# abelxiaoxing/ImageClassification

Measured on AMD Instinct MI355X. Metric: images/sec (whole node) ResNet-50 bf16 224^2 training, higher is better.
Workload: dtype bf16; 1 GPU; resnet50 train step, synthetic 3x224x224, batch 256/GPU, AdamW, label smoothing 0.1, 1000 classes (BASELINE configs[1]); global_batch=256, parallelism=dp1

## Files before the change

### imageclassification_amd/csrc/loss_optim.hip

```cpp
#define ICAMD_STREAM_NT 1
#include "common.h"
#include "icamd_internal.h"

namespace {

__global__ __launch_bounds__(256) void softmax_xent_kernel(const bf16_t* __restrict__ logits, int ld, int B, int C,
                                                           const long long* __restrict__ y1, const long long* __restrict__ y2,
                                                           float lam, float smoothing, float gscale,
                                                           float* __restrict__ loss_rows, int* __restrict__ pred,
                                                           bf16_t* __restrict__ dlogits) {
  const int lane = threadIdx.x & 63;
  const int row = blockIdx.x * 4 + (threadIdx.x >> 6);
  if (row >= B) return;
  const bf16_t* x = logits + (long long)row * ld;
  float mx = -INFINITY;
  int amax = lane < C ? lane : 0;
  for (int c = lane; c < C; c += 64) {
    const float v = bf16_to_f32(x[c]);
    if (v > mx) { mx = v; amax = c; }
  }
#pragma unroll
  for (int o = 32; o > 0; o >>= 1) {
    const float om = __shfl_xor(mx, o, 64);
    const int oa = __shfl_xor(amax, o, 64);
    if (om > mx || (om == mx && oa < amax)) { mx = om; amax = oa; }
  }
  float se = 0.f, sx = 0.f;
  for (int c = lane; c < C; c += 64) {
    const float v = bf16_to_f32(x[c]);
    se += __expf(v - mx);
    sx += v;
  }
  se = wave_sum(se);
  sx = wave_sum(sx);
  const float lse = mx + __logf(se);
  const int t1 = (int)y1[row];
  const int t2 = (y2 != nullptr) ? (int)y2[row] : t1;
  const float on = 1.f - smoothing, off = smoothing / (float)C;
  const float lp1 = bf16_to_f32(x[t1]) - lse, lp2 = bf16_to_f32(x[t2]) - lse;
  const float sum_logp = sx - (float)C * lse;
  const float loss = -(off * sum_logp + on * (lam * lp1 + (1.f - lam) * lp2));
  if (lane == 0) {
    loss_rows[row] = loss;
    if (pred != nullptr) pred[row] = amax;
  }
  if (dlogits != nullptr) {
    bf16_t* d = dlogits + (long long)row * ld;
    const float inv = 1.f / se;
    for (int c = lane; c < ld; c += 64) {
      float g = 0.f;
      if (c < C) {
        const float pc = __expf(bf16_to_f32(x[c]) - mx) * inv;
        float t = off;
        if (c == t1) t += on * lam;
        if (c == t2) t += on * (1.f - lam);
        g = (pc - t) * gscale;
      }
      d[c] = f32_to_bf16(g);
    }
  }
}

__global__ __launch_bounds__(256) void step_metrics_kernel(const float* __restrict__ loss_rows,
                                                           const int* __restrict__ pred,
                                                           const long long* __restrict__ target, int B, int C,
                                                           float* __restrict__ loss_out, int* __restrict__ finite_out,
                                                           double* __restrict__ acc_f64, int* __restrict__ counts,
                                                           float* __restrict__ loss_log, int log_slot, int log_stride,
                                                           int respect_skip) {
  __shared__ double red[256];
  __shared__ int cred[256];
  __shared__ int s_finite;
  const bool have_loss = loss_rows != nullptr;
  if (have_loss) {
    double s = 0.0;
    for (int i = threadIdx.x; i < B; i += 256) s += (double)loss_rows[i];
    red[threadIdx.x] = s;
    __syncthreads();
    for (int o = 128; o > 0; o >>= 1) {
      if ((int)threadIdx.x < o) red[threadIdx.x] += red[threadIdx.x + o];
      __syncthreads();
    }
    if (threadIdx.x == 0) {
      const float mean = (float)(red[0] / (double)B);
      const int fin = isfinite(mean) ? 1 : 0;
      *loss_out = mean;
      *finite_out = fin;
      s_finite = fin;
      if (loss_log != nullptr) loss_log[log_slot] = mean;
    }
  } else if (threadIdx.x == 0) {
    s_finite = *finite_out;
  }
  __syncthreads();
  if (respect_skip & 2) return;
  if ((respect_skip & 1) && !s_finite) return;
  const bool add_loss = have_loss || (respect_skip & 4);
  if (pred == nullptr) {
    if (threadIdx.x == 0 && add_loss) { acc_f64[0] += (double)*loss_out; acc_f64[1] += 1.0; }
    return;
  }
  int correct = 0;
  for (int i = threadIdx.x; i < B; i += 256) {
    const int p = pred[i];
    const int t = (int)target[i];
    if (p == t) {
      ++correct;
      if (counts != nullptr && t >= 0 && t < C) atomicAdd(&counts[t], 1);
    } else if (counts != nullptr) {
      if (p >= 0 && p < C) atomicAdd(&counts[C + p], 1);
      if (t >= 0 && t < C) atomicAdd(&counts[2 * C + t], 1);
    }
  }
  cred[threadIdx.x] = correct;
  __syncthreads();
  for (int o = 128; o > 0; o >>= 1) {
    if ((int)threadIdx.x < o) cred[threadIdx.x] += cred[threadIdx.x + o];
    __syncthreads();
  }
  if (threadIdx.x == 0) {
    if (add_loss) { acc_f64[0] += (double)*loss_out; acc_f64[1] += 1.0; }
    acc_f64[2] += (double)((float)cred[0] / (float)B);
    if (loss_log != nullptr && log_stride > 0) loss_log[log_stride + log_slot] = (float)cred[0] / (float)B;
    acc_f64[3] += (double)cred[0];
    acc_f64[4] += (double)B;
  }
}

__global__ __launch_bounds__(256) void sumsq_partial_kernel(const float* __restrict__ g, long long n4, long long n,
                                                            double* __restrict__ partial) {
  __shared__ double red[4];
  const long long stride = (long long)gridDim.x * blockDim.x;
  double s = 0.0;
  for (long long i = (long long)blockIdx.x * blockDim.x + threadIdx.x; i < n4; i += stride) {
    const f32x4 v = ((const f32x4*)g)[i];
    s += (double)(v[0] * v[0] + v[1] * v[1]) + (double)(v[2] * v[2] + v[3] * v[3]);
  }
  if (blockIdx.x == 0 && threadIdx.x == 0)
    for (long long i = n4 * 4; i < n; ++i) s += (double)g[i] * (double)g[i];
  s = wave_sum_d(s);
  if ((threadIdx.x & 63) == 0) red[threadIdx.x >> 6] = s;
  __syncthreads();
  if (threadIdx.x == 0) partial[blockIdx.x] = red[0] + red[1] + red[2] + red[3];
}

__global__ void gradnorm_finalize_kernel(const double* __restrict__ partial, int nblk, float inv_scale, float max_norm,
                                         float* __restrict__ out) {
  if (threadIdx.x != 0 || blockIdx.x != 0) return;
  double s = 0.0;
  for (int i = 0; i < nblk; ++i) s += partial[i];
  const float norm = (float)sqrt(s) * inv_scale;
  out[0] = norm;
  float coef = 1.f;
  if (max_norm > 0.f) { coef = max_norm / (norm + 1e-6f); if (coef > 1.f) coef = 1.f; }
  out[1] = coef;
}

struct AdamArgs {
  float lr, wd, beta1, beta2, eps, gscale, ema_w;
  int step;
  int bias_correct;
};

__device__ __forceinline__ void bias_corrections(const AdamArgs& a, const int* __restrict__ skipped, float& bc1,
                                                 float& bc2_sqrt) {
  bc1 = 1.f; bc2_sqrt = 1.f;
  if (a.bias_correct) {
    int t = a.step - (skipped != nullptr ? *skipped : 0);
    if (t < 1) t = 1;
    bc1 = (float)(1.0 - pow((double)a.beta1, (double)t));
    bc2_sqrt = (float)sqrt(1.0 - pow((double)a.beta2, (double)t));
  }
}
__device__ __forceinline__ bool step_skipped(const int* __restrict__ finite_flag, int* __restrict__ skipped, int flags) {
  if (finite_flag == nullptr || *finite_flag != 0) return false;
  if (skipped != nullptr && !(flags & 2) && blockIdx.x == 0 && threadIdx.x == 0) *skipped += 1;
  return true;
}

__global__ __launch_bounds__(256) void adamw_ema_kernel(float* __restrict__ p, float* __restrict__ g, float* __restrict__ m,
                                                        float* __restrict__ v, float* __restrict__ ema,
                                                        bf16_t* __restrict__ shadow, long long n4, AdamArgs a,
                                                        const float* __restrict__ clip, const int* __restrict__ finite_flag,
                                                        int* __restrict__ skipped, int zero_grad) {
  if (step_skipped(finite_flag, skipped, zero_grad)) return;
  float bc1, bc2_sqrt;
  bias_corrections(a, skipped, bc1, bc2_sqrt);
  const float gs = a.gscale * (clip != nullptr ? clip[1] : 1.f);
  const float decay_mul = 1.f - a.lr * a.wd;
  const float step_size = a.lr / bc1;
  const long long stride = (long long)gridDim.x * blockDim.x;
  for (long long i = (long long)blockIdx.x * blockDim.x + threadIdx.x; i < n4; i += stride) {
    f32x4 pv = ld_stream((const f32x4*)p + i);
    f32x4 gv = ld_stream((const f32x4*)g + i);
    f32x4 mv = ld_stream((const f32x4*)m + i);
    f32x4 vv = ld_stream((const f32x4*)v + i);
#pragma unroll
    for (int e = 0; e < 4; ++e) {
      const float gg = gv[e] * gs;
      float pp = pv[e] * decay_mul;
      const float mm = mv[e] + (gg - mv[e]) * (1.f - a.beta1);
      const float v2 = vv[e] * a.beta2 + (1.f - a.beta2) * gg * gg;
      const float denom = sqrtf(v2) / bc2_sqrt + a.eps;
      pp = pp - step_size * (mm / denom);
      pv[e] = pp; mv[e] = mm; vv[e] = v2;
    }
    ((f32x4*)p)[i] = pv;
    ((f32x4*)m)[i] = mv;
    ((f32x4*)v)[i] = vv;
    if (zero_grad & 1) ((f32x4*)g)[i] = f32x4{0.f, 0.f, 0.f, 0.f};
    if (ema != nullptr) {
      f32x4 ev = ld_stream((const f32x4*)ema + i);
#pragma unroll
      for (int e = 0; e < 4; ++e) ev[e] = ev[e] + a.ema_w * (pv[e] - ev[e]);
      ((f32x4*)ema)[i] = ev;
    }
    if (shadow != nullptr) {
      u32x2 sv;
      sv[0] = pack_bf16x2(pv[0], pv[1]);
      sv[1] = pack_bf16x2(pv[2], pv[3]);
      ((u32x2*)shadow)[i] = sv;
    }
  }
}

__global__ __launch_bounds__(256) void grad_guard_kernel(float* __restrict__ g, long long n4, const int* __restrict__ finite_flag) {
  if (*finite_flag != 0) return;
  const long long stride = (long long)gridDim.x * blockDim.x;
  for (long long i = (long long)blockIdx.x * blockDim.x + threadIdx.x; i < n4; i += stride)
    ((f32x4*)g)[i] = f32x4{0.f, 0.f, 0.f, 0.f};
}

__global__ __launch_bounds__(256) void lerp_kernel(float* __restrict__ dst, const float* __restrict__ src, long long n,
                                                   float w, const int* __restrict__ finite_flag) {
  if (finite_flag != nullptr && *finite_flag == 0) return;
  const long long stride = (long long)gridDim.x * blockDim.x;
  if (w == 1.f) {
    for (long long i = (long long)blockIdx.x * blockDim.x + threadIdx.x; i < n; i += stride) dst[i] = src[i];
    return;
  }
  for (long long i = (long long)blockIdx.x * blockDim.x + threadIdx.x; i < n; i += stride)
    dst[i] = dst[i] + w * (src[i] - dst[i]);
}

__global__ __launch_bounds__(256) void f32_to_bf16_kernel(const float* __restrict__ src, bf16_t* __restrict__ dst,
                                                          long long n) {
  const long long stride = (long long)gridDim.x * blockDim.x;
  for (long long i = (long long)blockIdx.x * blockDim.x + threadIdx.x; i < n; i += stride) dst[i] = f32_to_bf16(src[i]);
}

__global__ __launch_bounds__(256) void filter_transpose_kernel(const bf16_t* __restrict__ src_base,
                                                               bf16_t* __restrict__ dst_base,
                                                               const long long* __restrict__ descs,
                                                               const int* __restrict__ jobs) {
  const int layer = jobs[blockIdx.x * 2 + 0];
  const int start = jobs[blockIdx.x * 2 + 1];
  const long long* d = descs + (long long)layer * 8;
  const bf16_t* src = src_base + d[0];
  bf16_t* dst = dst_base + d[1];
  const int Cout = (int)d[2], T = (int)d[3], Cin = (int)d[4];
  const int total = Cout * T * Cin;
  for (int k = 0; k < 16; ++k) {
    const int o = start + k * 256 + threadIdx.x;
    if (o < total) {
      const int co = o % Cout;
      const int rest = o / Cout;
      const int t = rest % T;
      const int ci = rest / T;
      dst[o] = src[((long long)co * T + t) * Cin + ci];
    }
  }
}

__global__ __launch_bounds__(256) void filter_transpose_tiled_kernel(const bf16_t* __restrict__ src_base,
                                                                     bf16_t* __restrict__ dst_base,
                                                                     const long long* __restrict__ descs,
                                                                     const int* __restrict__ jobs) {
  __shared__ bf16_t tile[64][72];
  const int* job = jobs + blockIdx.x * 4;
  const long long* d = descs + (long long)job[0] * 8;
  const int t = job[1], co0 = job[2], ci0 = job[3];
  const int Cout = (int)d[2], T = (int)d[3], Cin = (int)d[4];
  const bf16_t* src = src_base + d[0];
  bf16_t* dst = dst_base + d[1];
  const int r = threadIdx.x >> 3, c8 = (threadIdx.x & 7) * 8;
#pragma unroll
  for (int pass = 0; pass < 2; ++pass) {
    const int co = r + pass * 32;
    const u32x4 v = *(const u32x4*)(src + ((long long)(co0 + co) * T + t) * Cin + ci0 + c8);
    *(u32x4*)&tile[co][c8] = v;
  }
  __syncthreads();
#pragma unroll
  for (int pass = 0; pass < 2; ++pass) {
    const int ci = r + pass * 32;
    unsigned int w[4];
#pragma unroll
    for (int e = 0; e < 4; ++e)
      w[e] = (unsigned int)tile[c8 + 2 * e][ci] | ((unsigned int)tile[c8 + 2 * e + 1][ci] << 16);
    *(u32x4*)(dst + ((long long)(ci0 + ci) * T + t) * Cout + co0 + c8) = u32x4{w[0], w[1], w[2], w[3]};
  }
}

__global__ __launch_bounds__(256) void colsum_kernel(const bf16_t* __restrict__ x, int rows, int ld, int cols,
                                                     float* __restrict__ out, int accumulate) {
  const int c = blockIdx.x * blockDim.x + threadIdx.x;
  if (c >= cols) return;
  float s = 0.f;
  for (int r = 0; r < rows; ++r) s += bf16_to_f32(x[(long long)r * ld + c]);
  out[c] = accumulate ? out[c] + s : s;
}

inline unsigned int grid_for(long long work_items, int threads) {
  long long blocks = (work_items + threads - 1) / threads;
  if (blocks > 2048) blocks = 2048;
  if (blocks < 1) blocks = 1;
  return (unsigned int)blocks;
}

}

int icamd_softmax_xent_launch(const bf16_t* logits, int ld, int B, int C, const long long* y1, const long long* y2,
                              float lam, float smoothing, float gscale, float* loss_rows, int* pred, bf16_t* dlogits,
                              hipStream_t s) {
  if (B <= 0 || C <= 0 || ld < C) return ICAMD_ERR_BAD_ARG;
  hipLaunchKernelGGL(softmax_xent_kernel, dim3((unsigned)((B + 3) / 4)), dim3(256), 0, s, logits, ld, B, C, y1, y2, lam,
                     smoothing, gscale, loss_rows, pred, dlogits);
  return icamd_launch_status();
}

int icamd_step_metrics_launch(const float* loss_rows, const int* pred, const long long* target, int B, int C,
                              float* loss_out, int* finite_out, double* acc_f64, int* counts, float* loss_log,
                              int log_slot, int log_stride, int respect_skip, hipStream_t s) {
  hipLaunchKernelGGL(step_metrics_kernel, dim3(1), dim3(256), 0, s, loss_rows, pred, target, B, C, loss_out, finite_out,
                     acc_f64, counts, loss_log, log_slot, log_stride, respect_skip);
  return icamd_launch_status();
}

#define ICAMD_SUMSQ_BLOCKS 512
int icamd_grad_norm_launch(const float* g, long long n, float inv_scale, float max_norm, double* partial, float* out,
                           hipStream_t s) {
  const long long n4 = n / 4;
  hipLaunchKernelGGL(sumsq_partial_kernel, dim3(ICAMD_SUMSQ_BLOCKS), dim3(256), 0, s, g, n4, n, partial);
  hipLaunchKernelGGL(gradnorm_finalize_kernel, dim3(1), dim3(64), 0, s, partial, ICAMD_SUMSQ_BLOCKS, inv_scale, max_norm,
                     out);
  return icamd_launch_status();
}

int icamd_adamw_ema_launch(float* p, float* g, float* m, float* v, float* ema, bf16_t* shadow, long long n, float lr,
                           float wd, float beta1, float beta2, float eps, int step, float gscale, float ema_decay,
                           const float* clip, const int* finite_flag, int* skipped, int zero_grad, hipStream_t s) {
  if (n % 4 != 0 || step < 1) return ICAMD_ERR_BAD_ARG;
  AdamArgs a;
  a.lr = lr; a.wd = wd; a.beta1 = beta1; a.beta2 = beta2; a.eps = eps; a.gscale = gscale;
  a.step = step; a.bias_correct = 1;
  a.ema_w = 1.f - ema_decay;
  hipLaunchKernelGGL(adamw_ema_kernel, dim3(grid_for(n / 4, 256)), dim3(256), 0, s, p, g, m, v, ema, shadow, n / 4, a, clip,
                     finite_flag, skipped, zero_grad);
  return icamd_launch_status();
}

int icamd_grad_guard_launch(float* g, long long n, const int* finite_flag, hipStream_t s) {
  if (n % 4 != 0) return ICAMD_ERR_BAD_ARG;
  hipLaunchKernelGGL(grad_guard_kernel, dim3(grid_for(n / 4, 256)), dim3(256), 0, s, g, n / 4, finite_flag);
  return icamd_launch_status();
}

template <int KIND>
__global__ __launch_bounds__(256) void optim_ema_kernel(float* __restrict__ p, float* __restrict__ g, float* __restrict__ m,
                                                        float* __restrict__ v, float* __restrict__ ema,
                                                        bf16_t* __restrict__ shadow, long long n4, AdamArgs a,
                                                        const float* __restrict__ clip, const int* __restrict__ finite_flag,
                                                        int* __restrict__ skipped, int zero_grad) {
  if (step_skipped(finite_flag, skipped, zero_grad)) return;
  float bc1, bc2_sqrt;
  bias_corrections(a, skipped, bc1, bc2_sqrt);
  const float gs = a.gscale * (clip != nullptr ? clip[1] : 1.f);
  const float step_size = a.lr / bc1;
  const long long stride = (long long)gridDim.x * blockDim.x;
  for (long long i = (long long)blockIdx.x * blockDim.x + threadIdx.x; i < n4; i += stride) {
    f32x4 pv = ((f32x4*)p)[i];
    const f32x4 gv = ((const f32x4*)g)[i];
    f32x4 mv = ((f32x4*)m)[i];
    f32x4 vv = {0.f, 0.f, 0.f, 0.f};
    if (KIND == 1) vv = ((f32x4*)v)[i];
#pragma unroll
    for (int e = 0; e < 4; ++e) {
      float gg = gv[e] * gs;
      if (KIND == 1) {
        gg += a.wd * pv[e];
        const float mm = mv[e] + (gg - mv[e]) * (1.f - a.beta1);
        const float v2 = vv[e] * a.beta2 + (1.f - a.beta2) * gg * gg;
        pv[e] -= step_size * (mm / (sqrtf(v2) / bc2_sqrt + a.eps));
        mv[e] = mm; vv[e] = v2;
      } else if (KIND == 2 || KIND == 3) {
        gg += a.wd * pv[e];
        const float buf = a.beta1 * mv[e] + gg;
        pv[e] -= a.lr * (KIND == 3 ? gg + a.beta1 * buf : buf);
        mv[e] = buf;
      } else {
        const float u = mv[e] * a.beta1 + gg * (1.f - a.beta1);
        const float sg = u > 0.f ? 1.f : (u < 0.f ? -1.f : 0.f);
        pv[e] = pv[e] * (1.f - a.lr * a.wd) - a.lr * sg;
        mv[e] = mv[e] + (gg - mv[e]) * (1.f - a.beta2);
      }
    }
    ((f32x4*)p)[i] = pv;
    ((f32x4*)m)[i] = mv;
    if (KIND == 1) ((f32x4*)v)[i] = vv;
    if (zero_grad & 1) ((f32x4*)g)[i] = f32x4{0.f, 0.f, 0.f, 0.f};
    if (ema != nullptr) {
      f32x4 ev = ld_stream((const f32x4*)ema + i);
#pragma unroll
      for (int e = 0; e < 4; ++e) ev[e] = ev[e] + a.ema_w * (pv[e] - ev[e]);
      ((f32x4*)ema)[i] = ev;
    }
    if (shadow != nullptr) {
      u32x2 sv;
      sv[0] = pack_bf16x2(pv[0], pv[1]);
      sv[1] = pack_bf16x2(pv[2], pv[3]);
      ((u32x2*)shadow)[i] = sv;
    }
  }
}

int icamd_optim_ema_launch(int kind, float* p, float* g, float* m, float* v, float* ema, bf16_t* shadow, long long n,
                           float lr, float wd, float beta1, float beta2, float eps, int step, float gscale,
                           float ema_decay, const float* clip, const int* finite_flag, int* skipped, int zero_grad,
                           hipStream_t s) {
  if (kind == 0) return icamd_adamw_ema_launch(p, g, m, v, ema, shadow, n, lr, wd, beta1, beta2, eps, step, gscale, ema_decay,
                                               clip, finite_flag, skipped, zero_grad, s);
  if (n % 4 != 0 || step < 1 || kind < 0 || kind > 4 || (kind == 1 && v == nullptr)) return ICAMD_ERR_BAD_ARG;
  AdamArgs a;
  a.lr = lr; a.wd = wd; a.beta1 = beta1; a.beta2 = beta2; a.eps = eps; a.gscale = gscale;
  a.step = step; a.bias_correct = kind == 1 ? 1 : 0;
  a.ema_w = 1.f - ema_decay;
  const dim3 grid(grid_for(n / 4, 256)), block(256);
  if (kind == 1) hipLaunchKernelGGL(optim_ema_kernel<1>, grid, block, 0, s, p, g, m, v, ema, shadow, n / 4, a, clip, finite_flag, skipped, zero_grad);
  else if (kind == 2) hipLaunchKernelGGL(optim_ema_kernel<2>, grid, block, 0, s, p, g, m, v, ema, shadow, n / 4, a, clip, finite_flag, skipped, zero_grad);
  else if (kind == 3) hipLaunchKernelGGL(optim_ema_kernel<3>, grid, block, 0, s, p, g, m, v, ema, shadow, n / 4, a, clip, finite_flag, skipped, zero_grad);
  else hipLaunchKernelGGL(optim_ema_kernel<4>, grid, block, 0, s, p, g, m, v, ema, shadow, n / 4, a, clip, finite_flag, skipped, zero_grad);
  return icamd_launch_status();
}

int icamd_lerp_launch(float* dst, const float* src, long long n, float w, const int* finite_flag, hipStream_t s) {
  hipLaunchKernelGGL(lerp_kernel, dim3(grid_for(n, 256)), dim3(256), 0, s, dst, src, n, w, finite_flag);
  return icamd_launch_status();
}

int icamd_f32_to_bf16_launch(const float* src, bf16_t* dst, long long n, hipStream_t s) {
  hipLaunchKernelGGL(f32_to_bf16_kernel, dim3(grid_for(n, 256)), dim3(256), 0, s, src, dst, n);
  return icamd_launch_status();
}

int icamd_filter_transpose_launch(const bf16_t* src_base, bf16_t* dst_base, const long long* descs, const int* jobs,
                                  int njobs, hipStream_t s) {
  if (njobs <= 0) return ICAMD_OK;
  hipLaunchKernelGGL(filter_transpose_kernel, dim3((unsigned)njobs), dim3(256), 0, s, src_base, dst_base, descs, jobs);
  return icamd_launch_status();
}

int icamd_filter_transpose_tiled_launch(const bf16_t* src_base, bf16_t* dst_base, const long long* descs, const int* jobs,
                                        int njobs, hipStream_t s) {
  if (njobs <= 0) return ICAMD_OK;
  hipLaunchKernelGGL(filter_transpose_tiled_kernel, dim3((unsigned)njobs), dim3(256), 0, s, src_base, dst_base, descs, jobs);
  return icamd_launch_status();
}

int icamd_colsum_launch(const bf16_t* x, int rows, int ld, int cols, float* out, int accumulate, hipStream_t s) {
  hipLaunchKernelGGL(colsum_kernel, dim3((unsigned)((cols + 255) / 256)), dim3(256), 0, s, x, rows, ld, cols, out,
                     accumulate);
  return icamd_launch_status();
}
```

### imageclassification_amd/csrc/norm_pool.hip

```cpp
#include "common.h"
#include "icamd_internal.h"
#include <stdlib.h>
#include <string.h>

#ifndef ICAMD_BN_NT
#define ICAMD_BN_NT 1
#endif

namespace {

__device__ __forceinline__ u32x4 bn_ld(const void* base, long long i) {
  if constexpr (ICAMD_BN_NT & 1) return __builtin_nontemporal_load((const u32x4*)base + i);
  else return ((const u32x4*)base)[i];
}
__device__ __forceinline__ void bn_st(void* base, long long i, const u32x4 v) {
  if constexpr (ICAMD_BN_NT & 2) __builtin_nontemporal_store(v, (u32x4*)base + i);
  else ((u32x4*)base)[i] = v;
}

__global__ void bn_eval_coeffs_kernel(int C, const float* __restrict__ gamma, const float* __restrict__ beta,
                                      const float* __restrict__ running_mean, const float* __restrict__ running_var,
                                      float eps, float* __restrict__ scale_out, float* __restrict__ shift_out) {
  const int c = blockIdx.x * blockDim.x + threadIdx.x;
  if (c >= C) return;
  const float invstd = 1.0f / sqrtf(running_var[c] + eps);
  const float sc = gamma[c] * invstd;
  scale_out[c] = sc;
  shift_out[c] = beta[c] - running_mean[c] * sc;
}

struct BnFinalizeArgs {
  const float* gamma; const float* beta; float* running_mean; float* running_var;
  float momentum, eps;
  float* mean_out; float* invstd_out; float* scale_out; float* shift_out;
  float* dgamma; float* dbeta; float* c1_out; float* c2_out; int accumulate;
  const float* gy_mean; const float* gy_invstd;
  double count;
};

template <int MODE, int CG>
__global__ __launch_bounds__(1024) void bn_reduce_finalize_kernel(const float* __restrict__ part, double* __restrict__ chunks,
                                                                  unsigned int* __restrict__ counters, int nrows, int C,
                                                                  int rows_per_chunk, BnFinalizeArgs a) {
  constexpr int RL = 1024 / CG;
  __shared__ double red[RL][2][CG];
  __shared__ int s_last;
  const int cc = threadIdx.x & (CG - 1);
  const int c = blockIdx.x * CG + cc;
  const int rl = threadIdx.x / CG;
  const int r0 = blockIdx.y * rows_per_chunk;
  const int r1 = min(nrows, r0 + rows_per_chunk);
  double s1 = 0.0, s2 = 0.0;
  if (c < C) {
    double u1 = 0.0, u2 = 0.0;
    int r = r0 + rl;
    constexpr int UN = 8;
    for (; r + (2 * UN - 1) * RL < r1; r += 2 * UN * RL) {
      float a0[UN], a1[UN], b0[UN], b1[UN];
#pragma unroll
      for (int k = 0; k < UN; ++k) {
        a0[k] = part[((long long)(r + 2 * k * RL) * 2 + 0) * C + c];
        a1[k] = part[((long long)(r + 2 * k * RL) * 2 + 1) * C + c];
        b0[k] = part[((long long)(r + (2 * k + 1) * RL) * 2 + 0) * C + c];
        b1[k] = part[((long long)(r + (2 * k + 1) * RL) * 2 + 1) * C + c];
      }
#pragma unroll
      for (int k = 0; k < UN; ++k) { s1 += (double)a0[k]; s2 += (double)a1[k]; u1 += (double)b0[k]; u2 += (double)b1[k]; }
    }
    for (; r + RL < r1; r += 2 * RL) {
      const float a0 = part[((long long)r * 2 + 0) * C + c], a1 = part[((long long)r * 2 + 1) * C + c];
      const float b0 = part[((long long)(r + RL) * 2 + 0) * C + c], b1 = part[((long long)(r + RL) * 2 + 1) * C + c];
      s1 += (double)a0; s2 += (double)a1; u1 += (double)b0; u2 += (double)b1;
    }
    if (r < r1) { s1 += (double)part[((long long)r * 2 + 0) * C + c]; s2 += (double)part[((long long)r * 2 + 1) * C + c]; }
    s1 += u1; s2 += u2;
  }
  red[rl][0][cc] = s1;
  red[rl][1][cc] = s2;
  __syncthreads();
  double t1 = 0.0, t2 = 0.0;
  if (gridDim.y == 1) {
    if (threadIdx.x >= CG || c >= C) return;
#pragma unroll
    for (int j = 0; j < RL; ++j) { t1 += red[j][0][cc]; t2 += red[j][1][cc]; }
  } else {
  if (threadIdx.x < 2 * CG) {
    const int which = threadIdx.x / CG;
    double s = 0.0;
#pragma unroll
    for (int j = 0; j < RL; ++j) s += red[j][which][cc];
    if (c < C) chunks[((long long)blockIdx.y * 2 + which) * C + c] = s;
  }
  asm volatile("s_waitcnt vmcnt(0)" ::: "memory");
  __syncthreads();
  if (threadIdx.x == 0) {
    __builtin_amdgcn_fence(__ATOMIC_RELEASE, "agent");
    asm volatile("s_waitcnt vmcnt(0)" ::: "memory");
    const unsigned int prev = __hip_atomic_fetch_add(&counters[blockIdx.x], 1u, __ATOMIC_RELAXED, __HIP_MEMORY_SCOPE_AGENT);
    const int last = (prev == gridDim.y - 1) ? 1 : 0;
    if (last) {
      __builtin_amdgcn_fence(__ATOMIC_ACQUIRE, "agent");
      asm volatile("s_waitcnt vmcnt(0)" ::: "memory");
      __hip_atomic_store(&counters[blockIdx.x], 0u, __ATOMIC_RELAXED, __HIP_MEMORY_SCOPE_AGENT);
    }
    s_last = last;
  }
  __syncthreads();
  if (!s_last) return;
  const int nchunks = gridDim.y;
  double p1 = 0.0, p2 = 0.0;
  if (c < C) {
    for (int k = rl; k < nchunks; k += RL) {
      p1 += chunks[((long long)k * 2 + 0) * C + c];
      p2 += chunks[((long long)k * 2 + 1) * C + c];
    }
  }
  red[rl][0][cc] = p1;
  red[rl][1][cc] = p2;
  __syncthreads();
  if (threadIdx.x >= CG || c >= C) return;
#pragma unroll
  for (int j = 0; j < RL; ++j) { t1 += red[j][0][cc]; t2 += red[j][1][cc]; }
  }
  if constexpr (MODE == 0) {
    const double mean = t1 / a.count;
    double var = t2 / a.count - mean * mean;
    if (var < 0.0) var = 0.0;
    const float invstd = (float)(1.0 / sqrt(var + (double)a.eps));
    const float meanf = (float)mean;
    a.mean_out[c] = meanf;
    a.invstd_out[c] = invstd;
    const float sc = a.gamma[c] * invstd;
    a.scale_out[c] = sc;
    a.shift_out[c] = a.beta[c] - meanf * sc;
    if (a.running_mean != nullptr) {
      const double unbiased = a.count > 1.0 ? var * (a.count / (a.count - 1.0)) : var;
      a.running_mean[c] = (1.f - a.momentum) * a.running_mean[c] + a.momentum * meanf;
      a.running_var[c] = (1.f - a.momentum) * a.running_var[c] + a.momentum * (float)unbiased;
    }
  } else {
    if (a.gy_mean != nullptr) t2 = (double)a.gy_invstd[c] * (t2 - (double)a.gy_mean[c] * t1);
    a.c1_out[c] = (float)(t1 / a.count);
    a.c2_out[c] = (float)(t2 / a.count);
    if (a.accumulate) { a.dgamma[c] += (float)t2; a.dbeta[c] += (float)t1; }
    else { a.dgamma[c] = (float)t2; a.dbeta[c] = (float)t1; }
  }
}

__global__ __launch_bounds__(256) void bn_apply_kernel(const bf16_t* __restrict__ y, const float* __restrict__ scale,
                                                       const float* __restrict__ shift, const bf16_t* __restrict__ residual,
                                                       bf16_t* __restrict__ out, unsigned char* __restrict__ maskbits,
                                                       long long nvec, int cpr, int relu,
                                                       const float* __restrict__ res_scale,
                                                       const float* __restrict__ res_shift) {
  const long long stride = (long long)gridDim.x * blockDim.x;
  long long i = (long long)blockIdx.x * blockDim.x + threadIdx.x;
  const int cg = (int)(i % cpr) * 8;
  float sc[8], sh[8], rsc[8], rsh[8];
#pragma unroll
  for (int e = 0; e < 8; ++e) { sc[e] = scale[cg + e]; sh[e] = shift[cg + e]; }
  const bool res_bn = res_scale != nullptr;
#pragma unroll
  for (int e = 0; e < 8; ++e) { rsc[e] = res_bn ? res_scale[cg + e] : 1.f; rsh[e] = res_bn ? res_shift[cg + e] : 0.f; }
  for (; i < nvec; i += stride) {
    const u32x4 v = bn_ld(y, i);
    float f[8];
#pragma unroll
    for (int e = 0; e < 4; ++e) {
      f[2 * e] = fmaf(bf16_lo(v[e]), sc[2 * e], sh[2 * e]);
      f[2 * e + 1] = fmaf(bf16_hi(v[e]), sc[2 * e + 1], sh[2 * e + 1]);
    }
    if (residual != nullptr) {
      const u32x4 r = bn_ld(residual, i);
      if (res_bn) {
#pragma unroll
        for (int e = 0; e < 4; ++e) {
          f[2 * e] += bf16_to_f32(f32_to_bf16(fmaf(bf16_lo(r[e]), rsc[2 * e], rsh[2 * e])));
          f[2 * e + 1] += bf16_to_f32(f32_to_bf16(fmaf(bf16_hi(r[e]), rsc[2 * e + 1], rsh[2 * e + 1])));
        }
      } else {
#pragma unroll
        for (int e = 0; e < 4; ++e) { f[2 * e] += bf16_lo(r[e]); f[2 * e + 1] += bf16_hi(r[e]); }
      }
    }
    if (relu) {
#pragma unroll
      for (int e = 0; e < 8; ++e) f[e] = (f[e] < 0.f) ? 0.f : f[e];
    }
    u32x4 o;
#pragma unroll
    for (int e = 0; e < 4; ++e) o[e] = pack_bf16x2(f[2 * e], f[2 * e + 1]);
    bn_st(out, i, o);
    if (maskbits != nullptr) {
      unsigned int bits = 0;
#pragma unroll
      for (int e = 0; e < 8; ++e) bits |= (f[e] > 0.f ? 1u : 0u) << e;
      maskbits[i] = (unsigned char)bits;
    }
  }
}

struct PoolGather {
  const unsigned char* idx;
  int IH, IW, OH, OW;
  FastDiv dIW, dIH;
};

__device__ __forceinline__ u32x4 pool_gather8(const bf16_t* __restrict__ dout, const PoolGather& pg, unsigned int row,
                                              unsigned int cpr, unsigned int cg) {
  const unsigned int t1 = fdiv(row, pg.dIW);
  const int w = (int)(row - t1 * pg.IW);
  const unsigned int n = fdiv(t1, pg.dIH);
  const int h = (int)(t1 - n * pg.IH);
  float acc[8];
#pragma unroll
  for (int e = 0; e < 8; ++e) acc[e] = 0.f;
  const int oh_lo = h >> 1, oh_hi = (h + 1) >> 1, ow_lo = w >> 1, ow_hi = (w + 1) >> 1;
  for (int oh = oh_lo; oh <= oh_hi; ++oh) {
    if (oh >= pg.OH) continue;
    const int r = h - (oh * 2 - 1);
    for (int ow = ow_lo; ow <= ow_hi; ++ow) {
      if (ow >= pg.OW) continue;
      const unsigned int code4 = (unsigned)(r * 3 + (w - (ow * 2 - 1))) * 0x01010101u;
      const unsigned int o = ((n * pg.OH + oh) * pg.OW + ow) * cpr + cg;
      const u32x2 iv = ((const u32x2*)pg.idx)[o];
      const u32x4 d = ((const u32x4*)dout)[o];
      const unsigned int m0 = iv[0] ^ code4, m1 = iv[1] ^ code4;
#pragma unroll
      for (int e = 0; e < 8; ++e) {
        const unsigned int mb = ((e < 4 ? m0 : m1) >> ((e & 3) * 8)) & 0xffu;
        const float dv = (e & 1) ? bf16_hi(d[e >> 1]) : bf16_lo(d[e >> 1]);
        acc[e] += mb == 0u ? dv : 0.f;
      }
    }
  }
  u32x4 out;
#pragma unroll
  for (int e = 0; e < 4; ++e) out[e] = pack_bf16x2(acc[2 * e], acc[2 * e + 1]);
  return out;
}

__global__ __launch_bounds__(256) void bn_bwd_reduce_kernel(const bf16_t* __restrict__ dout, const bf16_t* __restrict__ act,
                                                            const bf16_t* __restrict__ y, const float* __restrict__ mean,
                                                            const float* __restrict__ invstd, const float* __restrict__ scale,
                                                            const float* __restrict__ shift, float* __restrict__ part,
                                                            const unsigned char* __restrict__ maskbits, long long rows, int C,
                                                            int rows_per_block, int relu, const PoolGather pg) {
  __shared__ float red[256 * 16];
  const int cpr = C >> 3;
  const int tid = threadIdx.x;
  const long long r0 = (long long)blockIdx.x * rows_per_block;
  const long long r1 = (rows < r0 + rows_per_block) ? rows : r0 + rows_per_block;
  for (int cg0 = 0; cg0 < cpr; cg0 += 256) {
    const int tcols = (cpr - cg0 < 256) ? (cpr - cg0) : 256;
    const int rlanes = 256 / tcols;
    const int cgi = tid % tcols, rl = tid / tcols;
    float sg[8], sgx[8];
#pragma unroll
    for (int e = 0; e < 8; ++e) { sg[e] = 0.f; sgx[e] = 0.f; }
    if (rl < rlanes) {
      const int c = (cg0 + cgi) * 8;
      float mu[8], is[8], sc[8], sh[8];
#pragma unroll
      for (int e = 0; e < 8; ++e) { mu[e] = mean[c + e]; is[e] = invstd[c + e]; sc[e] = scale[c + e]; sh[e] = shift[c + e]; }
      for (long long r = r0 + rl; r < r1; r += rlanes) {
        const long long off = r * cpr + cg0 + cgi;
        const u32x4 d = pg.idx != nullptr ? pool_gather8(dout, pg, (unsigned)r, (unsigned)cpr, (unsigned)(cg0 + cgi))
                                          : bn_ld(dout, off);
        const u32x4 yv = bn_ld(y, off);
        float g[8], yy[8];
#pragma unroll
        for (int e = 0; e < 4; ++e) {
          g[2 * e] = bf16_lo(d[e]); g[2 * e + 1] = bf16_hi(d[e]);
          yy[2 * e] = bf16_lo(yv[e]); yy[2 * e + 1] = bf16_hi(yv[e]);
        }
        if (relu) {
          if (maskbits != nullptr) {
            const unsigned int bits = maskbits[off];
#pragma unroll
            for (int e = 0; e < 8; ++e)
              if (!((bits >> e) & 1u)) g[e] = 0.f;
          } else if (act != nullptr) {
            const u32x4 a = bn_ld(act, off);
#pragma unroll
            for (int e = 0; e < 4; ++e) {
              if (!(bf16_lo(a[e]) > 0.f)) g[2 * e] = 0.f;
              if (!(bf16_hi(a[e]) > 0.f)) g[2 * e + 1] = 0.f;
            }
          } else {
#pragma unroll
            for (int e = 0; e < 8; ++e)
              if (!(fmaf(yy[e], sc[e], sh[e]) > 0.f)) g[e] = 0.f;
          }
        }
#pragma unroll
        for (int e = 0; e < 8; ++e) {
          sg[e] += g[e];
          sgx[e] += g[e] * ((yy[e] - mu[e]) * is[e]);
        }
      }
    }
#pragma unroll
    for (int e = 0; e < 8; ++e) { red[tid * 16 + e] = sg[e]; red[tid * 16 + 8 + e] = sgx[e]; }
    __syncthreads();
    for (int o = tid; o < tcols * 16; o += 256) {
      const int cgo = o >> 4, e = o & 15;
      float s = 0.f;
      for (int l = 0; l < rlanes; ++l) s += red[(l * tcols + cgo) * 16 + e];
      const int which = e >> 3;
      part[((long long)blockIdx.x * 2 + which) * C + (cg0 + cgo) * 8 + (e & 7)] = s;
    }
    __syncthreads();
  }
}

__global__ __launch_bounds__(256) void bn_bwd_apply_kernel(const bf16_t* __restrict__ dout, const bf16_t* __restrict__ act,
                                                           const bf16_t* __restrict__ y, const float* __restrict__ mean,
                                                           const float* __restrict__ invstd, const float* __restrict__ scale,
                                                           const float* __restrict__ shift, const float* __restrict__ c1,
                                                           const float* __restrict__ c2, bf16_t* __restrict__ dy,
                                                           bf16_t* __restrict__ gout, const unsigned char* __restrict__ maskbits,
                                                           long long nvec, int cpr, int relu, int reverse,
                                                           const PoolGather pg, const FastDiv dcpr) {
  const long long stride = (long long)gridDim.x * blockDim.x;
  long long k0 = (long long)blockIdx.x * blockDim.x + threadIdx.x;
  const int cg = (int)((reverse ? nvec - 1 - k0 : k0) % cpr) * 8;
  float mu[8], is[8], sc[8], sh[8], k1[8], k2[8];
#pragma unroll
  for (int e = 0; e < 8; ++e) {
    mu[e] = mean[cg + e]; is[e] = invstd[cg + e]; sc[e] = scale[cg + e]; sh[e] = shift[cg + e];
    k1[e] = c1[cg + e]; k2[e] = c2[cg + e];
  }
  for (; k0 < nvec; k0 += stride) {
    const long long i = reverse ? nvec - 1 - k0 : k0;
    u32x4 d;
    if (pg.idx != nullptr) {
      const unsigned int row = fdiv((unsigned)i, dcpr);
      d = pool_gather8(dout, pg, row, (unsigned)cpr, (unsigned)i - row * (unsigned)cpr);
    } else {
      d = bn_ld(dout, i);
    }
    const u32x4 yv = bn_ld(y, i);
    float g[8], yy[8];
#pragma unroll
    for (int e = 0; e < 4; ++e) {
      g[2 * e] = bf16_lo(d[e]); g[2 * e + 1] = bf16_hi(d[e]);
      yy[2 * e] = bf16_lo(yv[e]); yy[2 * e + 1] = bf16_hi(yv[e]);
    }
    if (relu) {
      if (maskbits != nullptr) {
        const unsigned int bits = maskbits[i];
#pragma unroll
        for (int e = 0; e < 8; ++e)
          if (!((bits >> e) & 1u)) g[e] = 0.f;
      } else if (act != nullptr) {
        const u32x4 a = bn_ld(act, i);
#pragma unroll
        for (int e = 0; e < 4; ++e) {
          if (!(bf16_lo(a[e]) > 0.f)) g[2 * e] = 0.f;
          if (!(bf16_hi(a[e]) > 0.f)) g[2 * e + 1] = 0.f;
        }
      } else {
#pragma unroll
        for (int e = 0; e < 8; ++e)
          if (!(fmaf(yy[e], sc[e], sh[e]) > 0.f)) g[e] = 0.f;
      }
    }
    float o[8];
#pragma unroll
    for (int e = 0; e < 8; ++e) o[e] = sc[e] * (g[e] - k1[e] - ((yy[e] - mu[e]) * is[e]) * k2[e]);
    u32x4 ov;
#pragma unroll
    for (int e = 0; e < 4; ++e) ov[e] = pack_bf16x2(o[2 * e], o[2 * e + 1]);
    bn_st(dy, i, ov);
    if (gout != nullptr) {
      u32x4 gv;
#pragma unroll
      for (int e = 0; e < 4; ++e) gv[e] = pack_bf16x2(g[2 * e], g[2 * e + 1]);
      bn_st(gout, i, gv);
    }
  }
}

__global__ __launch_bounds__(256) void bn_bwd_dual_reduce_kernel(const bf16_t* __restrict__ dout,
                                                                 const unsigned char* __restrict__ maskbits,
                                                                 const bf16_t* __restrict__ yA, const float* __restrict__ meanA,
                                                                 const float* __restrict__ invstdA,
                                                                 const bf16_t* __restrict__ yB, const float* __restrict__ meanB,
                                                                 const float* __restrict__ invstdB, float* __restrict__ partA,
                                                                 float* __restrict__ partB, long long rows, int C,
                                                                 int rows_per_block) {
  __shared__ float red[256 * 24];
  const int cpr = C >> 3;
  const int tid = threadIdx.x;
  const long long r0 = (long long)blockIdx.x * rows_per_block;
  const long long r1 = (rows < r0 + rows_per_block) ? rows : r0 + rows_per_block;
  for (int cg0 = 0; cg0 < cpr; cg0 += 256) {
    const int tcols = (cpr - cg0 < 256) ? (cpr - cg0) : 256;
    const int rlanes = 256 / tcols;
    const int cgi = tid % tcols, rl = tid / tcols;
    float sg[8], sa[8], sb[8];
#pragma unroll
    for (int e = 0; e < 8; ++e) { sg[e] = 0.f; sa[e] = 0.f; sb[e] = 0.f; }
    if (rl < rlanes) {
      const int c = (cg0 + cgi) * 8;
      float muA[8], isA[8], muB[8], isB[8];
#pragma unroll
      for (int e = 0; e < 8; ++e) { muA[e] = meanA[c + e]; isA[e] = invstdA[c + e]; muB[e] = meanB[c + e]; isB[e] = invstdB[c + e]; }
      for (long long r = r0 + rl; r < r1; r += rlanes) {
        const long long off = r * cpr + cg0 + cgi;
        const u32x4 d = bn_ld(dout, off);
        const u32x4 va = bn_ld(yA, off);
        const u32x4 vb = bn_ld(yB, off);
        const unsigned int bits = maskbits[off];
#pragma unroll
        for (int e = 0; e < 8; ++e) {
          const unsigned int wd = d[e >> 1], wa = va[e >> 1], wb = vb[e >> 1];
          float g = (e & 1) ? bf16_hi(wd) : bf16_lo(wd);
          if (!((bits >> e) & 1u)) g = 0.f;
          const float ya = (e & 1) ? bf16_hi(wa) : bf16_lo(wa), yb = (e & 1) ? bf16_hi(wb) : bf16_lo(wb);
          sg[e] += g;
          sa[e] += g * ((ya - muA[e]) * isA[e]);
          sb[e] += g * ((yb - muB[e]) * isB[e]);
        }
      }
    }
#pragma unroll
    for (int e = 0; e < 8; ++e) { red[tid * 24 + e] = sg[e]; red[tid * 24 + 8 + e] = sa[e]; red[tid * 24 + 16 + e] = sb[e]; }
    __syncthreads();
    for (int o = tid; o < tcols * 24; o += 256) {
      const int cgo = o / 24, e = o - cgo * 24;
      float s = 0.f;
      for (int l = 0; l < rlanes; ++l) s += red[(l * tcols + cgo) * 24 + e];
      const int ch = (cg0 + cgo) * 8 + (e & 7);
      if (e < 8) {
        partA[((long long)blockIdx.x * 2 + 0) * C + ch] = s;
        partB[((long long)blockIdx.x * 2 + 0) * C + ch] = s;
      } else if (e < 16) {
        partA[((long long)blockIdx.x * 2 + 1) * C + ch] = s;
      } else {
        partB[((long long)blockIdx.x * 2 + 1) * C + ch] = s;
      }
    }
    __syncthreads();
  }
}

__global__ __launch_bounds__(256) void bn_bwd_dual_apply_kernel(const bf16_t* __restrict__ dout,
                                                                const unsigned char* __restrict__ maskbits,
                                                                const bf16_t* __restrict__ yA, const float* __restrict__ meanA,
                                                                const float* __restrict__ invstdA, const float* __restrict__ scaleA,
                                                                const float* __restrict__ cA, bf16_t* __restrict__ dyA,
                                                                const bf16_t* __restrict__ yB, const float* __restrict__ meanB,
                                                                const float* __restrict__ invstdB, const float* __restrict__ scaleB,
                                                                const float* __restrict__ cB, bf16_t* __restrict__ dyB,
                                                                long long nvec, int cpr, int C, int reverse) {
  const long long stride = (long long)gridDim.x * blockDim.x;
  long long k0 = (long long)blockIdx.x * blockDim.x + threadIdx.x;
  const int cg = (int)((reverse ? nvec - 1 - k0 : k0) % cpr) * 8;
  float muA[8], isA[8], scA[8], k1A[8], k2A[8], muB[8], isB[8], scB[8], k1B[8], k2B[8];
#pragma unroll
  for (int e = 0; e < 8; ++e) {
    muA[e] = meanA[cg + e]; isA[e] = invstdA[cg + e]; scA[e] = scaleA[cg + e]; k1A[e] = cA[cg + e]; k2A[e] = cA[C + cg + e];
    muB[e] = meanB[cg + e]; isB[e] = invstdB[cg + e]; scB[e] = scaleB[cg + e]; k1B[e] = cB[cg + e]; k2B[e] = cB[C + cg + e];
  }
  for (; k0 < nvec; k0 += stride) {
    const long long i = reverse ? nvec - 1 - k0 : k0;
    const u32x4 d = bn_ld(dout, i);
    const u32x4 va = bn_ld(yA, i);
    const u32x4 vb = bn_ld(yB, i);
    const unsigned int bits = maskbits[i];
    float oa[8], ob[8];
#pragma unroll
    for (int e = 0; e < 8; ++e) {
      const unsigned int wd = d[e >> 1], wa = va[e >> 1], wb = vb[e >> 1];
      float g = (e & 1) ? bf16_hi(wd) : bf16_lo(wd);
      if (!((bits >> e) & 1u)) g = 0.f;
      const float ya = (e & 1) ? bf16_hi(wa) : bf16_lo(wa), yb = (e & 1) ? bf16_hi(wb) : bf16_lo(wb);
      oa[e] = scA[e] * (g - k1A[e] - ((ya - muA[e]) * isA[e]) * k2A[e]);
      ob[e] = scB[e] * (g - k1B[e] - ((yb - muB[e]) * isB[e]) * k2B[e]);
    }
    u32x4 pa, pb;
#pragma unroll
    for (int e = 0; e < 4; ++e) { pa[e] = pack_bf16x2(oa[2 * e], oa[2 * e + 1]); pb[e] = pack_bf16x2(ob[2 * e], ob[2 * e + 1]); }
    bn_st(dyA, i, pa);
    bn_st(dyB, i, pb);
  }
}

struct PoolDivs { FastDiv cpr, ow, oh; };

template <bool BNRELU>
__global__ __launch_bounds__(256) void maxpool3x3s2_fwd_kernel(const bf16_t* __restrict__ x, bf16_t* __restrict__ out,
                                                               unsigned char* __restrict__ idx, int N, int IH, int IW,
                                                               int C, int OH, int OW, const float* __restrict__ scale,
                                                               const float* __restrict__ shift, const PoolDivs dv) {
  const unsigned int cpr = (unsigned)C >> 3;
  const unsigned int total = (unsigned)N * OH * OW * cpr;
  const unsigned int stride = gridDim.x * blockDim.x;
  unsigned int i = blockIdx.x * blockDim.x + threadIdx.x;
  const unsigned int cg = i - fdiv(i, dv.cpr) * cpr;
  float sc[8], sh[8];
  if constexpr (BNRELU) {
#pragma unroll
    for (int e = 0; e < 8; ++e) { sc[e] = scale[cg * 8 + e]; sh[e] = shift[cg * 8 + e]; }
  }
  for (; i < total; i += stride) {
    unsigned int t = fdiv(i, dv.cpr);
    const unsigned int t1 = fdiv(t, dv.ow);
    const int ow = (int)(t - t1 * OW);
    const unsigned int n = fdiv(t1, dv.oh);
    const int oh = (int)(t1 - n * OH);
    if constexpr (BNRELU) {
      unsigned int key[8];
#pragma unroll
      for (int e = 0; e < 8; ++e) key[e] = 0u;
#pragma unroll
      for (int r = 0; r < 3; ++r) {
        const int ih = oh * 2 - 1 + r;
        if ((unsigned)ih >= (unsigned)IH) continue;
#pragma unroll
        for (int s = 0; s < 3; ++s) {
          const int iw = ow * 2 - 1 + s;
          if ((unsigned)iw >= (unsigned)IW) continue;
          const u32x4 v = ((const u32x4*)x)[((n * IH + ih) * IW + iw) * cpr + cg];
#pragma unroll
          for (int e = 0; e < 4; ++e) {
            float a0 = fmaf(bf16_lo(v[e]), sc[2 * e], sh[2 * e]);
            float a1 = fmaf(bf16_hi(v[e]), sc[2 * e + 1], sh[2 * e + 1]);
            a0 = a0 < 0.f ? 0.f : a0;
            a1 = a1 < 0.f ? 0.f : a1;
            const unsigned int pk = pack_bf16x2(a0, a1) & 0x7fff7fffu;
            const unsigned int k0 = ((pk & 0xffffu) << 8) | (unsigned)(15 - (r * 3 + s));
            const unsigned int k1 = ((pk >> 16) << 8) | (unsigned)(15 - (r * 3 + s));
            key[2 * e] = key[2 * e] > k0 ? key[2 * e] : k0;
            key[2 * e + 1] = key[2 * e + 1] > k1 ? key[2 * e + 1] : k1;
          }
        }
      }
      u32x4 o;
#pragma unroll
      for (int e = 0; e < 4; ++e) o[e] = ((key[2 * e] >> 8) & 0xffffu) | ((key[2 * e + 1] >> 8) << 16);
      ((u32x4*)out)[i] = o;
      if (idx != nullptr) {
        u32x2 iv;
        iv[0] = (15u - (key[0] & 15u)) | ((15u - (key[1] & 15u)) << 8) | ((15u - (key[2] & 15u)) << 16) | ((15u - (key[3] & 15u)) << 24);
        iv[1] = (15u - (key[4] & 15u)) | ((15u - (key[5] & 15u)) << 8) | ((15u - (key[6] & 15u)) << 16) | ((15u - (key[7] & 15u)) << 24);
        ((u32x2*)idx)[i] = iv;
      }
    } else {
      float best[8];
      int bi[8];
#pragma unroll
      for (int e = 0; e < 8; ++e) { best[e] = -INFINITY; bi[e] = 0; }
      bool first = true;
#pragma unroll
      for (int r = 0; r < 3; ++r) {
        const int ih = oh * 2 - 1 + r;
        if ((unsigned)ih >= (unsigned)IH) continue;
#pragma unroll
        for (int s = 0; s < 3; ++s) {
          const int iw = ow * 2 - 1 + s;
          if ((unsigned)iw >= (unsigned)IW) continue;
          const u32x4 v = ((const u32x4*)x)[((n * IH + ih) * IW + iw) * cpr + cg];
          float f[8];
#pragma unroll
          for (int e = 0; e < 4; ++e) { f[2 * e] = bf16_lo(v[e]); f[2 * e + 1] = bf16_hi(v[e]); }
#pragma unroll
          for (int e = 0; e < 8; ++e) {
            if (first || f[e] > best[e] || f[e] != f[e]) { best[e] = f[e]; bi[e] = r * 3 + s; }
          }
          first = false;
        }
      }
      u32x4 o;
#pragma unroll
      for (int e = 0; e < 4; ++e) o[e] = pack_bf16x2(best[2 * e], best[2 * e + 1]);
      ((u32x4*)out)[i] = o;
      if (idx != nullptr) {
        u32x2 iv;
        iv[0] = bi[0] | (bi[1] << 8) | (bi[2] << 16) | (bi[3] << 24);
        iv[1] = bi[4] | (bi[5] << 8) | (bi[6] << 16) | (bi[7] << 24);
        ((u32x2*)idx)[i] = iv;
      }
    }
  }
}

__global__ __launch_bounds__(256) void maxpool3x3s2_bwd_kernel(const bf16_t* __restrict__ dout,
                                                               const unsigned char* __restrict__ idx,
                                                               bf16_t* __restrict__ dx, int N, int IH, int IW, int C,
                                                               int OH, int OW, const PoolDivs dv) {
  const unsigned int cpr = (unsigned)C >> 3;
  const unsigned int total = (unsigned)N * IH * IW * cpr;
  const unsigned int stride = gridDim.x * blockDim.x;
  unsigned int i = blockIdx.x * blockDim.x + threadIdx.x;
  const unsigned int cg = i - fdiv(i, dv.cpr) * cpr;
  for (; i < total; i += stride) {
    const unsigned int t = fdiv(i, dv.cpr);
    const unsigned int t1 = fdiv(t, dv.ow);
    const int w = (int)(t - t1 * IW);
    const unsigned int n = fdiv(t1, dv.oh);
    const int h = (int)(t1 - n * IH);
    float acc[8];
#pragma unroll
    for (int e = 0; e < 8; ++e) acc[e] = 0.f;
    const int oh_lo = h >> 1, oh_hi = (h + 1) >> 1;
    const int ow_lo = w >> 1, ow_hi = (w + 1) >> 1;
    for (int oh = oh_lo; oh <= oh_hi; ++oh) {
      if (oh >= OH) continue;
      const int r = h - (oh * 2 - 1);
      for (int ow = ow_lo; ow <= ow_hi; ++ow) {
        if (ow >= OW) continue;
        const int s = w - (ow * 2 - 1);
        const unsigned int code4 = (unsigned)(r * 3 + s) * 0x01010101u;
        const unsigned int o = ((n * OH + oh) * OW + ow) * cpr + cg;
        const u32x2 iv = ((const u32x2*)idx)[o];
        const u32x4 d = ((const u32x4*)dout)[o];
        const unsigned int m0 = iv[0] ^ code4, m1 = iv[1] ^ code4;
#pragma unroll
        for (int e = 0; e < 8; ++e) {
          const unsigned int mb = ((e < 4 ? m0 : m1) >> ((e & 3) * 8)) & 0xffu;
          const float dvv = (e & 1) ? bf16_hi(d[e >> 1]) : bf16_lo(d[e >> 1]);
          acc[e] += mb == 0u ? dvv : 0.f;
        }
      }
    }
    u32x4 ov;
#pragma unroll
    for (int e = 0; e < 4; ++e) ov[e] = pack_bf16x2(acc[2 * e], acc[2 * e + 1]);
    ((u32x4*)dx)[i] = ov;
  }
}

__global__ __launch_bounds__(256) void avgpool_fwd_kernel(const bf16_t* __restrict__ x, bf16_t* __restrict__ out,
                                                          int N, int HW, int C) {
  const int cpr = C >> 3;
  const long long total = (long long)N * cpr;
  const long long i = (long long)blockIdx.x * blockDim.x + threadIdx.x;
  if (i >= total) return;
  const int cg = (int)(i % cpr);
  const int n = (int)(i / cpr);
  float acc[8];
#pragma unroll
  for (int e = 0; e < 8; ++e) acc[e] = 0.f;
  for (int p = 0; p < HW; ++p) {
    const u32x4 v = ((const u32x4*)x)[((long long)n * HW + p) * cpr + cg];
#pragma unroll
    for (int e = 0; e < 4; ++e) { acc[2 * e] += bf16_lo(v[e]); acc[2 * e + 1] += bf16_hi(v[e]); }
  }
  const float inv = 1.0f / (float)HW;
  u32x4 o;
#pragma unroll
  for (int e = 0; e < 4; ++e) o[e] = pack_bf16x2(acc[2 * e] * inv, acc[2 * e + 1] * inv);
  ((u32x4*)out)[i] = o;
}

__global__ __launch_bounds__(256) void avgpool_bwd_kernel(const bf16_t* __restrict__ dout, bf16_t* __restrict__ dx,
                                                          int N, int HW, int C) {
  const int cpr = C >> 3;
  const long long total = (long long)N * HW * cpr;
  const long long stride = (long long)gridDim.x * blockDim.x;
  const float inv = 1.0f / (float)HW;
  for (long long i = (long long)blockIdx.x * blockDim.x + threadIdx.x; i < total; i += stride) {
    const int cg = (int)(i % cpr);
    const int n = (int)(i / ((long long)HW * cpr));
    const u32x4 d = ((const u32x4*)dout)[(long long)n * cpr + cg];
    u32x4 o;
#pragma unroll
    for (int e = 0; e < 4; ++e) o[e] = pack_bf16x2(bf16_lo(d[e]) * inv, bf16_hi(d[e]) * inv);
    ((u32x4*)dx)[i] = o;
  }
}

__global__ __launch_bounds__(256) void pack_input_kernel(const float* __restrict__ x, bf16_t* __restrict__ out, int B,
                                                         int Cin, int H, int W, int mode, float lam, int yl, int yh,
                                                         int xl, int xh) {
  const long long total = (long long)B * H * W;
  const long long stride = (long long)gridDim.x * blockDim.x;
  const long long hw = (long long)H * W;
  for (long long i = (long long)blockIdx.x * blockDim.x + threadIdx.x; i < total; i += stride) {
    const int b = (int)(i / hw);
    const long long pix = i - (long long)b * hw;
    const int h = (int)(pix / W), w = (int)(pix - (long long)h * W);
    float f[8];
#pragma unroll
    for (int c = 0; c < 8; ++c) f[c] = 0.f;
    const int fb = B - 1 - b;
    for (int c = 0; c < Cin; ++c) {
      float v = x[((long long)b * Cin + c) * hw + pix];
      if (mode == 1) {
        const float o = x[((long long)fb * Cin + c) * hw + pix];
        v = v * lam + o * (1.f - lam);
      } else if (mode == 2) {
        if (h >= yl && h < yh && w >= xl && w < xh) v = x[((long long)fb * Cin + c) * hw + pix];
      }
      f[c] = v;
    }
    u32x4 o;
#pragma unroll
    for (int e = 0; e < 4; ++e) o[e] = pack_bf16x2(f[2 * e], f[2 * e + 1]);
    ((u32x4*)out)[i] = o;
  }
}

__global__ __launch_bounds__(256) void pack_input_rgb4_kernel(const float* __restrict__ x, bf16_t* __restrict__ out, int B,
                                                              int Cin, int H, int W, int mode, float lam, int yl, int yh,
                                                              int xl, int xh) {
  const int Wp2 = (W + (W & 1) + 8) / 2;
  const long long total = (long long)B * H * Wp2;
  const long long stride = (long long)gridDim.x * blockDim.x;
  const long long hw = (long long)H * W;
  for (long long i = (long long)blockIdx.x * blockDim.x + threadIdx.x; i < total; i += stride) {
    const long long row = i / Wp2;
    const int pp = (int)(i - row * Wp2);
    const int b = (int)(row / H), h = (int)(row - (long long)b * H);
    const int fb = B - 1 - b;
    float f[8];
#pragma unroll
    for (int c = 0; c < 8; ++c) f[c] = 0.f;
#pragma unroll
    for (int e = 0; e < 2; ++e) {
      const int w = 2 * pp + e - 3;
      if (w >= 0 && w < W) {
        const long long pix = (long long)h * W + w;
        for (int c = 0; c < Cin; ++c) {
          float v = x[((long long)b * Cin + c) * hw + pix];
          if (mode == 1) {
            const float o = x[((long long)fb * Cin + c) * hw + pix];
            v = v * lam + o * (1.f - lam);
          } else if (mode == 2) {
            if (h >= yl && h < yh && w >= xl && w < xh) v = x[((long long)fb * Cin + c) * hw + pix];
          }
          f[4 * e + c] = v;
        }
      }
    }
    u32x4 o;
#pragma unroll
    for (int e = 0; e < 4; ++e) o[e] = pack_bf16x2(f[2 * e], f[2 * e + 1]);
    ((u32x4*)out)[i] = o;
  }
}

inline unsigned int grid_for(long long work_items, int threads, int multiple_of) {
  static const long long cap = []() { const char* e = getenv("ICAMD_EW_BLOCKS"); return e ? atoll(e) : 1024ll; }();
  long long blocks = (work_items + threads - 1) / threads;
  if (blocks > cap) blocks = cap;
  if (blocks < 1) blocks = 1;
  if (multiple_of > 1) blocks = (blocks + multiple_of - 1) / multiple_of * multiple_of;
  return (unsigned int)blocks;
}
inline int bn_reverse() {
  static const int v = []() { const char* e = getenv("ICAMD_BN_REVERSE"); return e ? atoi(e) : 0; }();
  return v;
}
inline int gcd_i(int a, int b) { while (b) { int t = a % b; a = b; b = t; } return a; }

}


static void chunking(int nrows, int* rows_per_chunk, int* nchunks) {
  int rpc = 128;
  int nc = (nrows + rpc - 1) / rpc;
  if (nrows <= 512) { rpc = nrows > 0 ? nrows : 1; nc = 1; }
  if (nc > 64) { rpc = (nrows + 63) / 64; nc = (nrows + rpc - 1) / rpc; }
  *rows_per_chunk = rpc; *nchunks = nc;
}

static unsigned int* counters_of(double* chunks, int C) { (void)C; return (unsigned int*)((char*)chunks - 256); }

template <int MODE>
static void launch_reduce_finalize(const float* part, double* chunks, int nrows, int C, int rpc, int nc, const BnFinalizeArgs& a,
                                   hipStream_t s) {
  if (C <= 2048)
    hipLaunchKernelGGL((bn_reduce_finalize_kernel<MODE, 32>), dim3((unsigned)((C + 31) / 32), (unsigned)nc), dim3(1024), 0, s, part,
                       chunks, counters_of(chunks, C), nrows, C, rpc, a);
  else
    hipLaunchKernelGGL((bn_reduce_finalize_kernel<MODE, 64>), dim3((unsigned)((C + 63) / 64), (unsigned)nc), dim3(1024), 0, s, part,
                       chunks, counters_of(chunks, C), nrows, C, rpc, a);
}

int icamd_bn_finalize_launch(const float* part, int nrows, int C, double count, const float* gamma, const float* beta,
                             float* running_mean, float* running_var, float momentum, float eps, float* mean,
                             float* invstd, float* scale, float* shift, double* chunks, hipStream_t s) {
  int rpc, nc;
  chunking(nrows, &rpc, &nc);
  BnFinalizeArgs a = {};
  a.gamma = gamma; a.beta = beta; a.running_mean = running_mean; a.running_var = running_var;
  a.momentum = momentum; a.eps = eps; a.mean_out = mean; a.invstd_out = invstd; a.scale_out = scale; a.shift_out = shift;
  a.count = count;
  launch_reduce_finalize<0>(part, chunks, nrows, C, rpc, nc, a, s);
  return icamd_launch_status();
}

int icamd_sum_partials_launch(const float* part, int nrows, int C, float* out1, float* out2, int accumulate, double* chunks,
                              float* c1c2, hipStream_t s) {
  int rpc, nc;
  chunking(nrows, &rpc, &nc);
  BnFinalizeArgs a = {};
  a.dgamma = out2; a.dbeta = out1; a.c1_out = c1c2; a.c2_out = c1c2 + C; a.accumulate = accumulate; a.count = 1.0;
  launch_reduce_finalize<1>(part, chunks, nrows, C, rpc, nc, a, s);
  return icamd_launch_status();
}

int icamd_bn_eval_coeffs_launch(int C, const float* gamma, const float* beta, const float* rm, const float* rv, float eps,
                                float* scale, float* shift, hipStream_t s) {
  hipLaunchKernelGGL(bn_eval_coeffs_kernel, dim3((unsigned)((C + 255) / 256)), dim3(256), 0, s, C, gamma, beta, rm, rv,
                     eps, scale, shift);
  return icamd_launch_status();
}

static unsigned int elementwise_grid(long long nvec, int cpr) {
  const int mult = cpr / gcd_i(cpr, 256);
  return grid_for(nvec, 256, mult);
}

int icamd_bn_apply_launch(const bf16_t* y, const float* scale, const float* shift, const bf16_t* residual, bf16_t* out,
                          unsigned char* maskbits, long long numel, int C, int relu, hipStream_t s,
                          const float* res_scale, const float* res_shift) {
  if (C % 8 != 0 || numel % C != 0) return ICAMD_ERR_BAD_ARG;
  const long long nvec = numel / 8;
  const int cpr = C / 8;
  hipLaunchKernelGGL(bn_apply_kernel, dim3(elementwise_grid(nvec, cpr)), dim3(256), 0, s, y, scale, shift, residual, out,
                     maskbits, nvec, cpr, relu, res_scale, res_shift);
  return icamd_launch_status();
}

int icamd_bn_bwd_rows_per_block(long long rows, int C) {
  static const long long nb = []() { const char* e = getenv("ICAMD_BNBWD_BLOCKS"); return e ? atoll(e) : 1024ll; }();
  long long rpb = (rows + nb - 1) / nb;
  if (rpb < 32) rpb = 32;
  (void)C;
  return (int)rpb;
}

int icamd_bn_bwd_launch(const bf16_t* dout, const bf16_t* act, const bf16_t* y, const float* mean, const float* invstd,
                        const float* scale, const float* shift, float* dgamma, float* dbeta, bf16_t* dy, bf16_t* gout,
                        const unsigned char* maskbits, long long rows, int C, int relu, int accumulate, float* part,
                        double* chunks, float* c1c2, hipStream_t s, const unsigned char* pool_idx, int pool_ih, int pool_iw) {
  if (C % 8 != 0) return ICAMD_ERR_BAD_ARG;
  PoolGather pg;
  memset(&pg, 0, sizeof(pg));
  if (pool_idx != nullptr) {
    if (rows * (C / 8) >= (1ll << 31) || pool_ih < 1 || pool_iw < 1 || rows % ((long long)pool_ih * pool_iw) != 0)
      return ICAMD_ERR_BAD_ARG;
    pg.idx = pool_idx; pg.IH = pool_ih; pg.IW = pool_iw; pg.OH = (pool_ih - 1) / 2 + 1; pg.OW = (pool_iw - 1) / 2 + 1;
    pg.dIW = make_fastdiv((unsigned)pool_iw); pg.dIH = make_fastdiv((unsigned)pool_ih);
  }
  const FastDiv dcpr = make_fastdiv((unsigned)(C / 8));
  const int rpb = icamd_bn_bwd_rows_per_block(rows, C);
  const int nblk = (int)((rows + rpb - 1) / rpb);
  hipLaunchKernelGGL(bn_bwd_reduce_kernel, dim3((unsigned)nblk), dim3(256), 0, s, dout, act, y, mean, invstd, scale, shift,
                     part, maskbits, rows, C, rpb, relu, pg);
  int rc = icamd_launch_status();
  if (rc) return rc;
  float* c1 = c1c2;
  float* c2 = c1c2 + C;
  {
    int rpc, nc;
    chunking(nblk, &rpc, &nc);
    BnFinalizeArgs a = {};
    a.dgamma = dgamma; a.dbeta = dbeta; a.c1_out = c1; a.c2_out = c2; a.accumulate = accumulate; a.count = (double)rows;
    launch_reduce_finalize<1>(part, chunks, nblk, C, rpc, nc, a, s);
    rc = icamd_launch_status();
    if (rc) return rc;
  }
  const long long nvec = rows * (C / 8);
  hipLaunchKernelGGL(bn_bwd_apply_kernel, dim3(elementwise_grid(nvec, C / 8)), dim3(256), 0, s, dout, act, y, mean, invstd,
                     scale, shift, c1, c2, dy, gout, maskbits, nvec, C / 8, relu, bn_reverse(), pg, dcpr);
  return icamd_launch_status();
}

int icamd_bn_bwd_dual_launch(const bf16_t* dout, const unsigned char* maskbits, const bf16_t* yA, const float* meanA,
                             const float* invstdA, const float* scaleA, float* dgammaA, float* dbetaA, bf16_t* dyA,
                             const bf16_t* yB, const float* meanB, const float* invstdB, const float* scaleB, float* dgammaB,
                             float* dbetaB, bf16_t* dyB, long long rows, int C, int accumulate, float* partA, double* chunksA,
                             float* cA, float* partB, double* chunksB, float* cB, hipStream_t s) {
  if (C % 8 != 0) return ICAMD_ERR_BAD_ARG;
  const int rpb = icamd_bn_bwd_rows_per_block(rows, C);
  const int nblk = (int)((rows + rpb - 1) / rpb);
  hipLaunchKernelGGL(bn_bwd_dual_reduce_kernel, dim3((unsigned)nblk), dim3(256), 0, s, dout, maskbits, yA, meanA, invstdA, yB,
                     meanB, invstdB, partA, partB, rows, C, rpb);
  int rc = icamd_launch_status();
  if (rc) return rc;
  int rpc, nc;
  chunking(nblk, &rpc, &nc);
  for (int which = 0; which < 2; ++which) {
    BnFinalizeArgs a = {};
    a.dgamma = which ? dgammaB : dgammaA; a.dbeta = which ? dbetaB : dbetaA;
    a.c1_out = which ? cB : cA; a.c2_out = (which ? cB : cA) + C; a.accumulate = accumulate; a.count = (double)rows;
    double* chunks = which ? chunksB : chunksA;
    launch_reduce_finalize<1>(which ? partB : partA, chunks, nblk, C, rpc, nc, a, s);
    rc = icamd_launch_status();
    if (rc) return rc;
  }
  const long long nvec = rows * (C / 8);
  hipLaunchKernelGGL(bn_bwd_dual_apply_kernel, dim3(elementwise_grid(nvec, C / 8)), dim3(256), 0, s, dout, maskbits, yA, meanA,
                     invstdA, scaleA, cA, dyA, yB, meanB, invstdB, scaleB, cB, dyB, nvec, C / 8, C, bn_reverse());
  return icamd_launch_status();
}

int icamd_bn_bwd_reduce_launch(const bf16_t* g, const bf16_t* y, const float* mean, const float* invstd, float* part, long long rows,
                               int C, int* nblk_out, hipStream_t s) {
  if (C % 8 != 0) return ICAMD_ERR_BAD_ARG;
  PoolGather pg;
  memset(&pg, 0, sizeof(pg));
  const int rpb = icamd_bn_bwd_rows_per_block(rows, C);
  const int nblk = (int)((rows + rpb - 1) / rpb);
  hipLaunchKernelGGL(bn_bwd_reduce_kernel, dim3((unsigned)nblk), dim3(256), 0, s, g, (const bf16_t*)nullptr, y, mean, invstd, mean, mean,
                     part, (const unsigned char*)nullptr, rows, C, rpb, 0, pg);
  *nblk_out = nblk;
  return icamd_launch_status();
}

int icamd_bn_bwd_finalize_launch(const float* part, int nrows, const float* mean, const float* invstd, float* dgamma, float* dbeta,
                                 long long rows, int C, int accumulate, double* chunks, float* c1c2, hipStream_t s, int sums_are_gy) {
  int rpc, nc;
  chunking(nrows, &rpc, &nc);
  BnFinalizeArgs a = {};
  a.dgamma = dgamma; a.dbeta = dbeta; a.c1_out = c1c2; a.c2_out = c1c2 + C; a.accumulate = accumulate; a.count = (double)rows;
  if (sums_are_gy) { a.gy_mean = mean; a.gy_invstd = invstd; }
  launch_reduce_finalize<1>(part, chunks, nrows, C, rpc, nc, a, s);
  return icamd_launch_status();
}

int icamd_bn_bwd_apply_launch(const float* part, int nrows, const bf16_t* g, const bf16_t* y, const float* mean,
                              const float* invstd, const float* scale, float* dgamma, float* dbeta, bf16_t* dy,
                              long long rows, int C, int accumulate, double* chunks, float* c1c2, hipStream_t s,
                              int sums_are_gy) {
  float* c1 = c1c2;
  float* c2 = c1c2 + C;
  int rc;
  {
    int rpc, nc;
    chunking(nrows, &rpc, &nc);
    BnFinalizeArgs a = {};
    a.dgamma = dgamma; a.dbeta = dbeta; a.c1_out = c1; a.c2_out = c2; a.accumulate = accumulate; a.count = (double)rows;
    if (sums_are_gy) { a.gy_mean = mean; a.gy_invstd = invstd; }
    launch_reduce_finalize<1>(part, chunks, nrows, C, rpc, nc, a, s);
    rc = icamd_launch_status();
    if (rc) return rc;
  }
  const long long nvec = rows * (C / 8);
  hipLaunchKernelGGL(bn_bwd_apply_kernel, dim3(elementwise_grid(nvec, C / 8)), dim3(256), 0, s, g, (const bf16_t*)nullptr, y,
                     mean, invstd, scale, scale, c1, c2, dy, (bf16_t*)nullptr, (const unsigned char*)nullptr, nvec, C / 8, 0, 0, PoolGather{}, make_fastdiv((unsigned)(C / 8)));
  return icamd_launch_status();
}

static PoolDivs pool_divs(int C, int W, int H) {
  PoolDivs d;
  d.cpr = make_fastdiv((unsigned)(C / 8)); d.ow = make_fastdiv((unsigned)W); d.oh = make_fastdiv((unsigned)H);
  return d;
}

int icamd_maxpool_fwd_launch(const bf16_t* x, bf16_t* out, unsigned char* idx, int N, int IH, int IW, int C, int OH, int OW,
                             hipStream_t s) {
  if (C % 8 != 0 || (long long)N * IH * IW * (C / 8) >= (1ll << 31)) return ICAMD_ERR_BAD_ARG;
  const long long total = (long long)N * OH * OW * (C / 8);
  hipLaunchKernelGGL(maxpool3x3s2_fwd_kernel<false>, dim3(elementwise_grid(total, C / 8) * 4), dim3(256), 0, s, x, out, idx, N,
                     IH, IW, C, OH, OW, nullptr, nullptr, pool_divs(C, OW, OH));
  return icamd_launch_status();
}

int icamd_bn_relu_maxpool_fwd_launch(const bf16_t* y, const float* scale, const float* shift, bf16_t* out, unsigned char* idx,
                                     int N, int IH, int IW, int C, int OH, int OW, hipStream_t s) {
  if (C % 8 != 0 || (long long)N * IH * IW * (C / 8) >= (1ll << 31)) return ICAMD_ERR_BAD_ARG;
  const long long total = (long long)N * OH * OW * (C / 8);
  hipLaunchKernelGGL(maxpool3x3s2_fwd_kernel<true>, dim3(elementwise_grid(total, C / 8) * 4), dim3(256), 0, s, y, out, idx, N,
                     IH, IW, C, OH, OW, scale, shift, pool_divs(C, OW, OH));
  return icamd_launch_status();
}

int icamd_maxpool_bwd_launch(const bf16_t* dout, const unsigned char* idx, bf16_t* dx, int N, int IH, int IW, int C, int OH,
                             int OW, hipStream_t s) {
  if (C % 8 != 0 || (long long)N * IH * IW * (C / 8) >= (1ll << 31)) return ICAMD_ERR_BAD_ARG;
  const long long total = (long long)N * IH * IW * (C / 8);
  hipLaunchKernelGGL(maxpool3x3s2_bwd_kernel, dim3(elementwise_grid(total, C / 8) * 4), dim3(256), 0, s, dout, idx, dx, N, IH,
                     IW, C, OH, OW, pool_divs(C, IW, IH));
  return icamd_launch_status();
}

int icamd_avgpool_fwd_launch(const bf16_t* x, bf16_t* out, int N, int HW, int C, hipStream_t s) {
  if (C % 8 != 0) return ICAMD_ERR_BAD_ARG;
  const long long total = (long long)N * (C / 8);
  hipLaunchKernelGGL(avgpool_fwd_kernel, dim3((unsigned)((total + 255) / 256)), dim3(256), 0, s, x, out, N, HW, C);
  return icamd_launch_status();
}

int icamd_avgpool_bwd_launch(const bf16_t* dout, bf16_t* dx, int N, int HW, int C, hipStream_t s) {
  if (C % 8 != 0) return ICAMD_ERR_BAD_ARG;
  const long long total = (long long)N * HW * (C / 8);
  hipLaunchKernelGGL(avgpool_bwd_kernel, dim3(grid_for(total, 256, 1)), dim3(256), 0, s, dout, dx, N, HW, C);
  return icamd_launch_status();
}

int icamd_pack_input_launch(const float* x, bf16_t* out, int B, int Cin, int H, int W, int mode, float lam, int yl, int yh,
                            int xl, int xh, hipStream_t s) {
  if (Cin < 1 || Cin > 8) return ICAMD_ERR_BAD_ARG;
  const long long total = (long long)B * H * W;
  hipLaunchKernelGGL(pack_input_kernel, dim3(grid_for(total, 256, 1) * 2), dim3(256), 0, s, x, out, B, Cin, H, W, mode, lam,
                     yl, yh, xl, xh);
  return icamd_launch_status();
}


int icamd_pack_input_rgb4_launch(const float* x, bf16_t* out, int B, int Cin, int H, int W, int mode, float lam, int yl,
                                 int yh, int xl, int xh, hipStream_t s) {
  if (Cin < 1 || Cin > 3) return ICAMD_ERR_BAD_ARG;
  const long long total = (long long)B * H * ((W + (W & 1) + 8) / 2);
  hipLaunchKernelGGL(pack_input_rgb4_kernel, dim3(grid_for(total, 256, 1) * 2), dim3(256), 0, s, x, out, B, Cin, H, W, mode,
                     lam, yl, yh, xl, xh);
  return icamd_launch_status();
}


namespace {
__global__ __launch_bounds__(256) void bn_fold_kernel(const float* __restrict__ w, const float* __restrict__ gamma,
                                                      const float* __restrict__ beta, const float* __restrict__ rm,
                                                      const float* __restrict__ rv, float eps, int K,
                                                      bf16_t* __restrict__ out, float* __restrict__ shift) {
  const int co = blockIdx.x;
  const float scale = gamma[co] / sqrtf(rv[co] + eps);
  if (threadIdx.x == 0) shift[co] = beta[co] - rm[co] * scale;
  const float* src = w + (long long)co * K;
  bf16_t* dst = out + (long long)co * K;
  for (int k = threadIdx.x; k < K; k += 256) dst[k] = f32_to_bf16(src[k] * scale);
}
}

int icamd_bn_fold_launch(const float* w, const float* gamma, const float* beta, const float* rm, const float* rv, float eps,
                         int Cout, int K, bf16_t* w_folded, float* shift, hipStream_t s) {
  hipLaunchKernelGGL(bn_fold_kernel, dim3((unsigned)Cout), dim3(256), 0, s, w, gamma, beta, rm, rv, eps, K, w_folded, shift);
  return icamd_launch_status();
}
```

### imageclassification_amd/nets.py

```python
import ctypes
import math
import os
from collections import OrderedDict

import torch

from . import hip
from .checkpoint import PicklableModel

BN_EPS = 1e-5
_FUSED_BNBWD = os.environ.get("ICAMD_FUSED_BNBWD", "0") == "1"
_WGRAD_STREAM = os.environ.get("ICAMD_WGRAD_STREAM", "1") != "0"
_DUAL_BNBWD = os.environ.get("ICAMD_DUAL_BNBWD", "1") != "0"
_SUB2_SHORTCUT = os.environ.get("ICAMD_SUB2_SHORTCUT", "1") != "0"
_FUSED_POOL_BWD = os.environ.get("ICAMD_FUSED_POOL_BWD", "0") == "1"
BN_MOMENTUM = 0.1

ARCHS = {
    "resnet18": ("basic", [2, 2, 2, 2]),
    "resnet34": ("basic", [3, 4, 6, 3]),
    "resnet50": ("bottleneck", [3, 4, 6, 3]),
}


def _align(n, a):
    return (n + a - 1) // a * a


class _Param:
    __slots__ = ("name", "offset", "numel", "torch_shape", "kind", "padded_shape")

    def __init__(self, name, offset, numel, torch_shape, kind, padded_shape):
        self.name, self.offset, self.numel = name, offset, numel
        self.torch_shape, self.kind, self.padded_shape = torch_shape, kind, padded_shape


class _Conv:

    def __init__(self, name, cin, cout, k, stride, pad, cin_p=None, cout_p=None, bias=False, k_p=None):
        self.name = name
        self.cin, self.cout, self.k, self.stride, self.pad = cin, cout, k, stride, pad
        self.cin_p = cin_p or cin
        self.cout_p = cout_p or cout
        self.k_p = k_p or k
        self.has_bias = bias
        self.w = None
        self.b = None
        self.wt_offset = None
        self.descs = {}

    def desc(self, N, IH, IW):
        key = (N, IH, IW)
        d = self.descs.get(key)
        if d is None:
            d = hip.conv_desc(N, IH, IW, self.cin_p, self.cout_p, self.k, self.k, self.stride, self.pad)
            self.descs[key] = d
        return d


class _BN:
    def __init__(self, name, c):
        self.name, self.c = name, c
        self.weight = self.bias = None
        self.buf_offset = None
        self.stat_offset = None


class ResNet(PicklableModel):

    def __init__(self, arch="resnet50", num_classes=1000, device="cuda", zero_init_last=True, seed=None):
        hip.require_gpu()
        self.lib = hip.load()
        self.arch = arch
        self.num_classes = num_classes
        self.device = torch.device(device)
        self.training = True
        self._fold_dirty = True
        self.fold_eval = os.environ.get("ICAMD_EVAL_FOLD", "1") != "0"
        block, layers = ARCHS[arch]
        self.block = block
        self.expansion = 4 if block == "bottleneck" else 1
        self.ncls_p = _align(num_classes, 64)
        self._build_graph(layers)
        self._allocate()
        self.num_batches_tracked = 0
        self._ws = {}
        self._streams_ready = False
        self.wgrad_side_stream = True
        self.grad_ready_hook = None
        self.init_weights(zero_init_last=zero_init_last, seed=seed)

    def _build_graph(self, layers):
        self.convs, self.bns = [], []
        self.stem_conv = self._conv("conv1", 3, 64, 7, 2, 3, cin_p=4, k_p=8)
        self.stem_bn = self._bn("bn1", 64)
        self.blocks = []
        inplanes = 64
        for li, (planes, nblocks) in enumerate(zip([64, 128, 256, 512], layers)):
            for bi in range(nblocks):
                stride = 2 if (bi == 0 and li > 0) else 1
                name = f"layer{li + 1}.{bi}"
                outplanes = planes * self.expansion
                blk = {"name": name, "stride": stride}
                if self.block == "bottleneck":
                    blk["convs"] = [self._conv(f"{name}.conv1", inplanes, planes, 1, 1, 0),
                                    self._conv(f"{name}.conv2", planes, planes, 3, stride, 1),
                                    self._conv(f"{name}.conv3", planes, outplanes, 1, 1, 0)]
                    blk["bns"] = [self._bn(f"{name}.bn1", planes), self._bn(f"{name}.bn2", planes),
                                  self._bn(f"{name}.bn3", outplanes)]
                else:
                    blk["convs"] = [self._conv(f"{name}.conv1", inplanes, planes, 3, stride, 1),
                                    self._conv(f"{name}.conv2", planes, planes, 3, 1, 1)]
                    blk["bns"] = [self._bn(f"{name}.bn1", planes), self._bn(f"{name}.bn2", planes)]
                if stride != 1 or inplanes != outplanes:
                    blk["down_conv"] = self._conv(f"{name}.downsample.0", inplanes, outplanes, 1, stride, 0)
                    blk["down_bn"] = self._bn(f"{name}.downsample.1", outplanes)
                self.blocks.append(blk)
                inplanes = outplanes
        self.feat_dim = inplanes
        self.fc = self._conv("fc", inplanes, self.num_classes, 1, 1, 0, cout_p=self.ncls_p, bias=True)

    def _conv(self, name, cin, cout, k, stride, pad, cin_p=None, cout_p=None, bias=False, k_p=None):
        c = _Conv(name, cin, cout, k, stride, pad, cin_p, cout_p, bias, k_p)
        self.convs.append(c)
        return c

    def _bn(self, name, c):
        b = _BN(name, c)
        self.bns.append(b)
        return b

    def _allocate(self):
        dev = self.device
        order = [self.stem_conv, self.stem_bn]
        for blk in self.blocks:
            for c, b in zip(blk["convs"], blk["bns"]):
                order += [c, b]
            if "down_conv" in blk:
                order += [blk["down_conv"], blk["down_bn"]]
        order.append(self.fc)
        self.params = OrderedDict()
        off = 0

        def add(name, torch_shape, kind, padded_shape):
            nonlocal off
            numel = 1
            for s in padded_shape:
                numel *= s
            p = _Param(name, off, numel, tuple(torch_shape), kind, tuple(padded_shape))
            self.params[name] = p
            off = _align(off + numel, 64)
            return p

        boff = 0
        soff = 0
        for m in order:
            if isinstance(m, _Conv):
                wname = m.name + ".weight"
                m.w = add(wname, (m.cout, m.cin, m.k, m.k), "conv", (m.cout_p, m.k_p, m.k_p, m.cin_p))
                if m.has_bias:
                    m.b = add(m.name + ".bias", (m.cout,), "vec", (m.cout_p,))
            else:
                m.weight = add(m.name + ".weight", (m.c,), "vec", (m.c,))
                m.bias = add(m.name + ".bias", (m.c,), "vec", (m.c,))
                m.buf_offset = boff
                boff = _align(boff + 2 * m.c, 64)
                m.stat_offset = soff
                soff = _align(soff + 4 * m.c, 64)
        self.n_params = off
        self.param_arena = torch.zeros(off, dtype=torch.float32, device=dev)
        self.grad_arena = torch.zeros(off, dtype=torch.float32, device=dev)
        self.shadow = torch.zeros(off, dtype=torch.bfloat16, device=dev)
        self.buffer_arena = torch.zeros(max(boff, 64), dtype=torch.float32, device=dev)
        self.stat_arena = torch.zeros(max(soff, 64), dtype=torch.float32, device=dev)
        toff = 0
        descs, jobs, tjobs = [], [], []
        for m in self.convs:
            if m is self.stem_conv:
                continue
            m.wt_offset = toff
            T = m.k * m.k
            descs.append([m.w.offset, toff, m.cout_p, T, m.cin_p, 0, 0, 0])
            if m.cout_p % 64 == 0 and m.cin_p % 64 == 0:
                for t in range(T):
                    for co0 in range(0, m.cout_p, 64):
                        for ci0 in range(0, m.cin_p, 64):
                            tjobs.append([len(descs) - 1, t, co0, ci0])
            else:
                for s in range(0, m.w.numel, 4096):
                    jobs.append([len(descs) - 1, s])
            toff = _align(toff + m.w.numel, 128)
        self.shadow_t = torch.zeros(toff, dtype=torch.bfloat16, device=dev)
        self._tr_descs = torch.tensor(descs, dtype=torch.int64, device=dev)
        self._tr_jobs = torch.tensor(jobs if jobs else [[0, 0]], dtype=torch.int32, device=dev)
        self._tr_njobs = len(jobs)
        self._tr_tjobs = torch.tensor(tjobs if tjobs else [[0, 0, 0, 0]], dtype=torch.int32, device=dev)
        self._tr_ntjobs = len(tjobs)

    def _ctor_kwargs(self):
        return {"arch": self.arch, "num_classes": self.num_classes}

    def init_weights(self, zero_init_last=True, seed=None):
        g = torch.Generator()
        if seed is not None:
            g.manual_seed(seed)
        else:
            g.manual_seed(torch.initial_seed() % (2 ** 63))
        sd = OrderedDict()
        for name, p in self.params.items():
            if p.kind == "conv" and not name.startswith("fc."):
                cout, cin, k, _ = p.torch_shape
                std = math.sqrt(2.0 / (cout * k * k))
                sd[name] = torch.randn(p.torch_shape, generator=g) * std
            elif name == "fc.weight":
                bound = 1.0 / math.sqrt(p.torch_shape[1])
                sd[name] = (torch.rand(p.torch_shape[0], p.torch_shape[1], generator=g) * 2 - 1) * bound
            elif name == "fc.bias":
                bound = 1.0 / math.sqrt(self.feat_dim)
                sd[name] = (torch.rand(p.torch_shape, generator=g) * 2 - 1) * bound
            elif name.endswith(".weight"):
                sd[name] = torch.ones(p.torch_shape)
            else:
                sd[name] = torch.zeros(p.torch_shape)
        if zero_init_last:
            for blk in self.blocks:
                sd[blk["bns"][-1].name + ".weight"].zero_()
        for b in self.bns:
            sd[b.name + ".running_mean"] = torch.zeros(b.c)
            sd[b.name + ".running_var"] = torch.ones(b.c)
            sd[b.name + ".num_batches_tracked"] = torch.tensor(0)
        self.load_state_dict(sd)

    def _to_arena_layout(self, p, t):
        t = t.detach().to(torch.float32).cpu()
        if p.kind == "conv":
            if t.dim() == 2:
                t = t[:, :, None, None]
            cout, cin, kh, kw = t.shape
            full = torch.zeros(p.padded_shape)
            full[:cout, :kh, :kw, :cin] = t.permute(0, 2, 3, 1)
            return full.flatten()
        full = torch.zeros(p.padded_shape)
        full[: t.numel()] = t.flatten()
        return full

    def _from_arena_layout(self, p, flat):
        t = flat.reshape(p.padded_shape)
        if p.kind == "conv":
            cout, cin, kh, kw = (tuple(p.torch_shape) + (1, 1))[:4]
            t = t[:cout, :kh, :kw, :cin].permute(0, 3, 1, 2).contiguous()
            if p.name == "fc.weight":
                t = t.reshape(cout, cin)
            return t
        return t[: p.torch_shape[0]].clone()

    def load_state_dict(self, sd, strict=True):
        host = self.param_arena.cpu()
        missing = []
        for name, p in self.params.items():
            if name not in sd:
                missing.append(name)
                continue
            host[p.offset:p.offset + p.numel] = self._to_arena_layout(p, sd[name])
        bufs = self.buffer_arena.cpu()
        for b in self.bns:
            for j, key in enumerate(("running_mean", "running_var")):
                k = f"{b.name}.{key}"
                if k in sd:
                    bufs[b.buf_offset + j * b.c: b.buf_offset + (j + 1) * b.c] = sd[k].detach().float().cpu()
                else:
                    missing.append(k)
        k = f"{self.bns[0].name}.num_batches_tracked"
        if k in sd:
            self.num_batches_tracked = int(sd[k])
        if strict and missing:
            raise KeyError(f"missing keys in state_dict: {missing[:5]}{'...' if len(missing) > 5 else ''}")
        self.param_arena.copy_(host)
        self.buffer_arena.copy_(bufs)
        self.refresh_shadow()
        self._fold_dirty = True
        return missing

    def state_dict(self):
        host = self.param_arena.cpu()
        bufs = self.buffer_arena.cpu()
        sd = OrderedDict()
        by_module = OrderedDict()
        for name, p in self.params.items():
            by_module.setdefault(name.rsplit(".", 1)[0], []).append(p)
        bn_by_name = {b.name: b for b in self.bns}
        for mod, plist in by_module.items():
            for p in plist:
                sd[p.name] = self._from_arena_layout(p, host[p.offset:p.offset + p.numel])
            if mod in bn_by_name:
                b = bn_by_name[mod]
                sd[mod + ".running_mean"] = bufs[b.buf_offset:b.buf_offset + b.c].clone()
                sd[mod + ".running_var"] = bufs[b.buf_offset + b.c:b.buf_offset + 2 * b.c].clone()
                sd[mod + ".num_batches_tracked"] = torch.tensor(self.num_batches_tracked)
        return sd

    def named_parameters(self):
        for name, p in self.params.items():
            yield name, self.param_arena[p.offset:p.offset + p.numel]

    def parameters(self):
        for _, v in self.named_parameters():
            yield v

    def grad_of(self, name):
        p = self.params[name]
        return self._from_arena_layout(p, self.grad_arena[p.offset:p.offset + p.numel].cpu())

    def refresh_shadow(self):
        s = hip.stream_ptr()
        hip.check(self.lib.icamd_f32_to_bf16(self.param_arena.data_ptr(), self.shadow.data_ptr(), self.n_params, s),
                  "f32_to_bf16")
        self.refresh_transposed()

    def refresh_transposed(self):
        s = hip.stream_ptr()
        if self._tr_ntjobs:
            hip.check(self.lib.icamd_filter_transpose_tiled(self.shadow.data_ptr(), self.shadow_t.data_ptr(),
                                                            self._tr_descs.data_ptr(), self._tr_tjobs.data_ptr(),
                                                            self._tr_ntjobs, s), "filter_transpose_tiled")
        if self._tr_njobs:
            hip.check(self.lib.icamd_filter_transpose(self.shadow.data_ptr(), self.shadow_t.data_ptr(),
                                                      self._tr_descs.data_ptr(), self._tr_jobs.data_ptr(), self._tr_njobs,
                                                      s), "filter_transpose")

    def train(self, mode=True):
        self.training = bool(mode)
        self._fold_dirty = True
        return self

    def fold_batchnorm(self):
        dev = self.device
        if getattr(self, "shadow_eval", None) is None:
            self.shadow_eval = torch.empty_like(self.shadow)
            self.eval_shift = torch.zeros(sum(b.c for b in self.bns), dtype=torch.float32, device=dev)
            off = 0
            for b in self.bns:
                b.shift_offset = off
                off += b.c
        s = hip.stream_ptr()
        pairs = [(self.stem_conv, self.stem_bn)]
        for blk in self.blocks:
            pairs += list(zip(blk["convs"], blk["bns"]))
            if "down_conv" in blk:
                pairs.append((blk["down_conv"], blk["down_bn"]))
        for conv, bn in pairs:
            rm = self.buffer_arena.data_ptr() + 4 * bn.buf_offset
            hip.check(self.lib.icamd_bn_fold_filters(self._pf(conv.w), self._pf(bn.weight), self._pf(bn.bias), rm,
                                                     rm + 4 * bn.c, BN_EPS, conv.cout_p, conv.w.numel // conv.cout_p,
                                                     self.shadow_eval.data_ptr() + 2 * conv.w.offset,
                                                     self.eval_shift.data_ptr() + 4 * bn.shift_offset, s), bn.name)
        self._fold_dirty = False

    def _conv_act_eval(self, conv, bn, x, N, IH, IW, out, residual, relu, s):
        d = conv.desc(N, IH, IW)
        if conv is self.stem_conv:
            hip.check(self.lib.icamd_stem7x7s2_fwd(x, self.shadow_eval.data_ptr() + 2 * conv.w.offset, out.data_ptr(),
                                                   self.eval_shift.data_ptr() + 4 * bn.shift_offset, None, int(relu), N, IH, IW,
                                                   conv.cout_p, s), conv.name)
            return d
        hip.check(self.lib.icamd_conv2d_fwd_act(ctypes.byref(d), x, self.shadow_eval.data_ptr() + 2 * conv.w.offset,
                                                out.data_ptr(), self.eval_shift.data_ptr() + 4 * bn.shift_offset, residual,
                                                int(relu), s), conv.name)
        return d

    def _forward_eval_folded(self, ws):
        lib = self.lib
        s = hip.stream_ptr()
        N, H, W = ws["N"], ws["H"], ws["Ws"]
        if self._fold_dirty:
            self.fold_batchnorm()
        d0 = self._conv_act_eval(self.stem_conv, self.stem_bn, ws["x8"].data_ptr(), N, H, W, ws["a0"], None, True, s)
        hip.check(lib.icamd_maxpool3x3s2_fwd(ws["a0"].data_ptr(), ws["p0"].data_ptr(), None, N, d0.OH, d0.OW, 64, s),
                  "maxpool")
        x = ws["p0"]
        h, w = x.shape[1], x.shape[2]
        for blk, b in zip(self.blocks, ws["blocks"]):
            if "down_conv" in blk:
                self._conv_act_eval(blk["down_conv"], blk["down_bn"], x.data_ptr(), N, h, w, b["ad"], None, False, s)
                idn = b["ad"]
            else:
                idn = x
            cur, ch, cw = x, h, w
            n = len(blk["convs"])
            for i, (conv, bn) in enumerate(zip(blk["convs"], blk["bns"])):
                d = self._conv_act_eval(conv, bn, cur.data_ptr(), N, ch, cw, b["a"][i],
                                        idn.data_ptr() if i == n - 1 else None, True, s)
                cur, ch, cw = b["a"][i], d.OH, d.OW
            x, h, w = cur, ch, cw
        hip.check(lib.icamd_avgpool_fwd(x.data_ptr(), ws["pooled"].data_ptr(), N, h * w, self.feat_dim, s), "avgpool")
        dfc = self.fc.desc(N, 1, 1)
        hip.check(lib.icamd_conv2d_fwd(ctypes.byref(dfc), ws["pooled"].data_ptr(), self._w(self.fc),
                                       ws["logits"].data_ptr(), self._pf(self.fc.b), None, None, s), "fc")
        return ws["logits"]

    def eval(self):
        return self.train(False)

    def to(self, *a, **k):
        return self

    def _workspace(self, N, H, W):
        key = (N, H, W)
        ws = self._ws.get(key)
        if ws is not None:
            return ws
        dev = self.device
        lib = self.lib
        ws = {"N": N, "H": H, "W": W}

        def act(n, h, w, c):
            return torch.empty(n, h, w, c, dtype=torch.bfloat16, device=dev)

        Ws = W + (W & 1)
        ws["Ws"] = Ws
        ws["x8"] = act(N, H, Ws + 8, 4)
        d0 = self.stem_conv.desc(N, H, Ws)
        ws["y0"] = act(N, d0.OH, d0.OW, 64)
        ws["a0"] = act(N, d0.OH, d0.OW, 64)
        PH, PW = (d0.OH - 1) // 2 + 1, (d0.OW - 1) // 2 + 1
        ws["p0"] = act(N, PH, PW, 64)
        ws["p0_idx"] = torch.empty(N, PH, PW, 64, dtype=torch.uint8, device=dev)
        max_act = max(ws["y0"].numel(), ws["x8"].numel())
        max_stats = lib.icamd_conv2d_stats_rows(ctypes.byref(d0)) * 2 * 64
        max_wg = lib.icamd_stem7x7s2_wgrad_workspace_bytes(N, H, Ws, 64)
        max_bnb = lib.icamd_bn_bwd_workspace_bytes(N * d0.OH * d0.OW, 64)
        h, w = PH, PW
        blocks_ws = []
        for blk in self.blocks:
            b = {}
            ih, iw = h, w
            ys, acts = [], []
            for ci, conv in enumerate(blk["convs"]):
                d = conv.desc(N, ih, iw)
                ys.append(act(N, d.OH, d.OW, conv.cout_p))
                acts.append(act(N, d.OH, d.OW, conv.cout_p))
                max_act = max(max_act, ys[-1].numel())
                max_stats = max(max_stats, lib.icamd_conv2d_stats_rows(ctypes.byref(d)) * 2 * conv.cout_p)
                max_wg = max(max_wg, lib.icamd_conv2d_wgrad_workspace_bytes(ctypes.byref(d)))
                max_bnb = max(max_bnb, lib.icamd_bn_bwd_workspace_bytes(N * d.OH * d.OW, conv.cout_p))
                ih, iw = d.OH, d.OW
            b["y"], b["a"] = ys, acts
            b["mask"] = torch.empty(acts[-1].numel() // 8, dtype=torch.uint8, device=dev)
            if "down_conv" in blk:
                dd = blk["down_conv"].desc(N, h, w)
                b["yd"] = act(N, dd.OH, dd.OW, blk["down_conv"].cout_p)
                b["ad"] = act(N, dd.OH, dd.OW, blk["down_conv"].cout_p)
                max_stats = max(max_stats, lib.icamd_conv2d_stats_rows(ctypes.byref(dd)) * 2 * blk["down_conv"].cout_p)
                max_wg = max(max_wg, lib.icamd_conv2d_wgrad_workspace_bytes(ctypes.byref(dd)))
                max_bnb = max(max_bnb, lib.icamd_bn_bwd_workspace_bytes(N * dd.OH * dd.OW, blk["down_conv"].cout_p))
            blocks_ws.append(b)
            h, w = ih, iw
        ws["blocks"] = blocks_ws
        ws["final_hw"] = (h, w)
        ws["pooled"] = torch.empty(N, self.feat_dim, dtype=torch.bfloat16, device=dev)
        ws["logits"] = torch.zeros(N, self.ncls_p, dtype=torch.bfloat16, device=dev)
        dfc = self.fc.desc(N, 1, 1)
        max_wg = max(max_wg, lib.icamd_conv2d_wgrad_workspace_bytes(ctypes.byref(dfc)))
        ws["stats"] = torch.empty(max_stats, dtype=torch.float32, device=dev)
        ws["bn_ws"] = torch.zeros(lib.icamd_bn_workspace_bytes(2048), dtype=torch.uint8, device=dev)
        ws["wgrad_ws"] = torch.empty(max_wg, dtype=torch.uint8, device=dev)
        ws["wgrad_ws_bytes"] = max_wg
        ws["bnb_part"] = torch.empty(max_stats + 4 * 2 * 2048, dtype=torch.float32, device=dev)
        ws["bna_ws_bytes"] = lib.icamd_bn_bwd_apply_workspace_bytes(2048)
        ws["bna_ws"] = torch.zeros(ws["bna_ws_bytes"], dtype=torch.uint8, device=dev)
        ws["bnb_ws"] = torch.zeros(max_bnb, dtype=torch.uint8, device=dev)
        ws["bnb_ws2"] = torch.zeros(max_bnb, dtype=torch.uint8, device=dev)
        ws["bnb_ws_bytes"] = max_bnb
        ws["max_act"] = max_act
        ws["loss_rows"] = torch.empty(N, dtype=torch.float32, device=dev)
        ws["pred"] = torch.empty(N, dtype=torch.int32, device=dev)
        ws["dlogits"] = torch.zeros(N, self.ncls_p, dtype=torch.bfloat16, device=dev)
        ws["dpooled"] = torch.empty(N, self.feat_dim, dtype=torch.bfloat16, device=dev)
        ws["scale_shift_eval"] = torch.empty(2 * 2048, dtype=torch.float32, device=dev)
        self._ws[key] = ws
        return ws

    def _grad_buffers(self, ws):
        if "gbuf" not in ws:
            n = ws["max_act"]
            ws["gbuf"] = [torch.empty(n, dtype=torch.bfloat16, device=self.device) for _ in range(8)]
        return ws["gbuf"]

    def _w(self, conv):
        return self.shadow.data_ptr() + 2 * conv.w.offset

    def _wt(self, conv):
        return self.shadow_t.data_ptr() + 2 * conv.wt_offset

    def _pf(self, p):
        return self.param_arena.data_ptr() + 4 * p.offset

    def _gf(self, p):
        return self.grad_arena.data_ptr() + 4 * p.offset

    def _conv_bn_fwd(self, ws, conv, bn, x, N, IH, IW, y, out, residual, relu, s, maskbits=None, res_bn=None, conv_launch=None):
        lib = self.lib
        d = conv.desc(N, IH, IW)
        st = self.stat_arena.data_ptr() + 4 * bn.stat_offset
        c = bn.c
        mean, invstd, scale, shift = st, st + 4 * c, st + 8 * c, st + 12 * c
        stem = conv is self.stem_conv

        def conv_fwd(stats_ptr):
            if conv_launch is not None:
                conv_launch(stats_ptr)
                return
            if stem:
                hip.check(lib.icamd_stem7x7s2_fwd(x, self._w(conv), y.data_ptr(), None, stats_ptr, 0, N, IH, IW, conv.cout_p, s),
                          conv.name)
            else:
                hip.check(lib.icamd_conv2d_fwd(ctypes.byref(d), x, self._w(conv), y.data_ptr(), None, None, stats_ptr, s),
                          conv.name)

        if self.training:
            stats = ws["stats"].data_ptr()
            conv_fwd(stats)
            rows = lib.icamd_conv2d_stats_rows(ctypes.byref(d))
            rm = self.buffer_arena.data_ptr() + 4 * bn.buf_offset
            hip.check(lib.icamd_bn_train_finalize(stats, rows, c, float(N * d.OH * d.OW), self._pf(bn.weight),
                                                  self._pf(bn.bias), rm, rm + 4 * c, BN_MOMENTUM, BN_EPS, mean, invstd,
                                                  scale, shift, ws["bn_ws"].data_ptr(), s), bn.name)
        else:
            conv_fwd(None)
            rm = self.buffer_arena.data_ptr() + 4 * bn.buf_offset
            scale = ws["scale_shift_eval"].data_ptr()
            shift = scale + 4 * 2048
            hip.check(lib.icamd_bn_eval_coeffs(c, self._pf(bn.weight), self._pf(bn.bias), rm, rm + 4 * c, BN_EPS, scale,
                                               shift, s), bn.name)
        if out is None:
            return d, scale, shift
        if res_bn is not None:
            hip.check(lib.icamd_bn_apply_res_bn(y.data_ptr(), scale, shift, residual, res_bn[0], res_bn[1], out.data_ptr(),
                                                maskbits, y.numel(), c, int(relu), s), bn.name)
            return d
        hip.check(lib.icamd_bn_apply(y.data_ptr(), scale, shift, residual, out.data_ptr(), maskbits, y.numel(), c, int(relu),
                                     s), bn.name)
        return d

    def pack(self, x_nchw, mix=None):
        N, C, H, W = x_nchw.shape
        ws = self._workspace(N, H, W)
        mode, lam, box = (0, 1.0, (0, 0, 0, 0)) if mix is None else mix
        hip.check(self.lib.icamd_pack_input_rgb4(x_nchw.data_ptr(), ws["x8"].data_ptr(), N, C, H, W, mode, float(lam),
                                                 int(box[0]), int(box[1]), int(box[2]), int(box[3]), hip.stream_ptr()), "pack")
        return ws

    def forward_packed(self, ws, logits_only=False):
        lib = self.lib
        s = hip.stream_ptr()
        N, H, W = ws["N"], ws["H"], ws["Ws"]
        if not self.training and self.fold_eval:
            return self._forward_eval_folded(ws)
        if self.training:
            self.num_batches_tracked += 1
        d0, sc0, sh0 = self._conv_bn_fwd(ws, self.stem_conv, self.stem_bn, ws["x8"].data_ptr(), N, H, W, ws["y0"], None, None,
                                         True, s)
        hip.check(lib.icamd_bn_relu_maxpool3x3s2_fwd(ws["y0"].data_ptr(), sc0, sh0, ws["p0"].data_ptr(),
                                                     ws["p0_idx"].data_ptr() if self.training else None, N, d0.OH, d0.OW, 64,
                                                     s), "stem bn+relu+maxpool")
        x = ws["p0"]
        h, w = x.shape[1], x.shape[2]
        pending = None
        nblocks = len(self.blocks)
        for bi, (blk, b) in enumerate(zip(self.blocks, ws["blocks"])):
            b["in"] = x
            b["in_hw"] = (h, w)
            convs, bns = blk["convs"], blk["bns"]
            first_done = False
            if pending is not None:
                pd = pending
                pending = None
                c0, bn0 = convs[0], bns[0]
                d0 = c0.desc(N, h, w)

                def launch(stats_ptr, pd=pd, c0=c0, d0=d0, b=b):
                    hip.check(lib.icamd_bn_apply_conv1x1_fused(ctypes.byref(d0), pd["y"].data_ptr(), pd["scale"], pd["shift"],
                                                               pd["res"], pd["res_scale"], pd["res_shift"], pd["out"].data_ptr(),
                                                               pd["mask"].data_ptr(), self._w(c0), b["y"][0].data_ptr(), stats_ptr, s),
                              pd["name"] + " apply + " + c0.name)

                self._conv_bn_fwd(ws, c0, bn0, x.data_ptr(), N, h, w, b["y"][0], b["a"][0], None, True, s, conv_launch=launch)
                first_done = True
            res_bn = None
            if "down_conv" in blk and self.training:
                _, scd, shd = self._conv_bn_fwd(ws, blk["down_conv"], blk["down_bn"], x.data_ptr(), N, h, w, b["yd"], None,
                                                None, False, s)
                idn, res_bn = b["yd"], (scd, shd)
            elif "down_conv" in blk:
                self._conv_bn_fwd(ws, blk["down_conv"], blk["down_bn"], x.data_ptr(), N, h, w, b["yd"], b["ad"], None,
                                  False, s)
                idn = b["ad"]
            else:
                idn = x
            cur, ch, cw = x, h, w
            for i, (conv, bn) in enumerate(zip(convs, bns)):
                last = i == len(convs) - 1
                if i == 0 and first_done:
                    d = conv.desc(N, ch, cw)
                    cur, ch, cw = b["a"][i], d.OH, d.OW
                    continue
                defer = False
                if last and self.training and self.block == "bottleneck" and bi + 1 < nblocks:
                    dn = self.blocks[bi + 1]["convs"][0].desc(N, ch, cw)
                    defer = bool(lib.icamd_bn_apply_conv1x1_fused_supported(ctypes.byref(dn)))
                if defer:
                    d, sc3, sh3 = self._conv_bn_fwd(ws, conv, bn, cur.data_ptr(), N, ch, cw, b["y"][i], None, None, True, s)
                    pending = {"y": b["y"][i], "scale": sc3, "shift": sh3, "res": idn.data_ptr(),
                               "res_scale": res_bn[0] if res_bn else None, "res_shift": res_bn[1] if res_bn else None,
                               "out": b["a"][i], "mask": b["mask"], "name": bn.name}
                else:
                    d = self._conv_bn_fwd(ws, conv, bn, cur.data_ptr(), N, ch, cw, b["y"][i], b["a"][i],
                                          idn.data_ptr() if last else None, True, s,
                                          b["mask"].data_ptr() if (last and self.training) else None,
                                          res_bn if last else None)
                cur, ch, cw = b["a"][i], d.OH, d.OW
            x, h, w = cur, ch, cw
        hip.check(lib.icamd_avgpool_fwd(x.data_ptr(), ws["pooled"].data_ptr(), N, h * w, self.feat_dim, s), "avgpool")
        dfc = self.fc.desc(N, 1, 1)
        hip.check(lib.icamd_conv2d_fwd(ctypes.byref(dfc), ws["pooled"].data_ptr(), self._w(self.fc),
                                       ws["logits"].data_ptr(), self._pf(self.fc.b), None, None, s), "fc")
        return ws["logits"]

    def __call__(self, x_nchw):
        ws = self.pack(x_nchw.to(self.device, dtype=torch.float32).contiguous())
        logits = self.forward_packed(ws)
        return logits[:, : self.num_classes]

    def backward_packed(self, ws, accumulate=False):
        if _FUSED_BNBWD:
            return self._backward_packed_fused(ws, accumulate)
        lib = self.lib
        main = torch.cuda.current_stream()
        s = main.cuda_stream
        N = ws["N"]
        acc = int(bool(accumulate))
        wsp, wsb = ws["wgrad_ws"].data_ptr(), ws["wgrad_ws_bytes"]
        bws, bwb = ws["bnb_ws"].data_ptr(), ws["bnb_ws_bytes"]
        bufs = self._grad_buffers(ws)
        D0, D1, T, DA = (b.data_ptr() for b in bufs[:4])
        ypool = [b.data_ptr() for b in bufs[4:]]
        hook = self.grad_ready_hook
        side = self._wgrad_stream() if (_WGRAD_STREAM and self.wgrad_side_stream) else None
        ws_side = side.cuda_stream if side is not None else s
        pending = [None] * len(ypool)
        state = {"next": 0, "last": None}

        def next_y():
            k = state["next"]
            state["next"] = (k + 1) % len(ypool)
            if pending[k] is not None:
                main.wait_event(pending[k])
                pending[k] = None
            return k

        def wgrad(conv, x_ptr, dy_ptr, n, ih, iw, ybuf=None):
            d = conv.desc(n, ih, iw)
            if side is not None:
                ready = torch.cuda.Event()
                ready.record(main)
                side.wait_event(ready)
            if conv is self.stem_conv:
                hip.check(lib.icamd_stem7x7s2_wgrad(x_ptr, dy_ptr, self._gf(conv.w), acc, wsp, wsb, n, ih, iw, conv.cout_p, ws_side),
                          conv.name + " wgrad")
            else:
                hip.check(lib.icamd_conv2d_wgrad(ctypes.byref(d), x_ptr, dy_ptr, self._gf(conv.w), acc, wsp, wsb, ws_side),
                          conv.name + " wgrad")
            if side is not None:
                done = torch.cuda.Event()
                done.record(side)
                state["last"] = done
                if ybuf is not None:
                    pending[ybuf] = done

        def join_side():
            if state["last"] is not None:
                main.wait_event(state["last"])
                state["last"] = None

        def side_events():
            return () if state["last"] is None else (state["last"],)

        def dgrad(conv, dy_ptr, dx_ptr, addend, n, ih, iw, addend_bits=None):
            d = conv.desc(n, ih, iw)
            hip.check(lib.icamd_conv2d_dgrad(ctypes.byref(d), dy_ptr, self._wt(conv), dx_ptr, addend, addend_bits, s),
                      conv.name + " dgrad")

        def bn_bwd(bn, dout_ptr, act_ptr, y, dy_ptr, gout_ptr, relu, maskbits=None):
            st = self.stat_arena.data_ptr() + 4 * bn.stat_offset
            c = bn.c
            rows = y.numel() // c
            hip.check(lib.icamd_bn_bwd(dout_ptr, act_ptr, y.data_ptr(), st, st + 4 * c, st + 8 * c, st + 12 * c,
                                       self._gf(bn.weight), self._gf(bn.bias), dy_ptr, gout_ptr, maskbits, rows, c, int(relu),
                                       acc, bws, bwb, s), bn.name + " bwd")

        dl = ws["dlogits"].data_ptr()
        wgrad(self.fc, ws["pooled"].data_ptr(), dl, N, 1, 1)
        hip.check(lib.icamd_colsum(dl, N, self.ncls_p, self.ncls_p, self._gf(self.fc.b), acc, s), "fc bias grad")
        dgrad(self.fc, dl, ws["dpooled"].data_ptr(), None, N, 1, 1)
        if hook:
            hook(self.fc.w.offset, self.n_params, side_events())
        fh, fw = ws["final_hw"]
        dout, other = D0, D1
        hip.check(lib.icamd_avgpool_bwd(ws["dpooled"].data_ptr(), dout, N, fh * fw, self.feat_dim, s), "avgpool bwd")

        fused_rows = 0
        for bi in range(len(self.blocks) - 1, -1, -1):
            blk, b = self.blocks[bi], ws["blocks"][bi]
            convs, bns = blk["convs"], blk["bns"]
            h, w = b["in_hw"]
            xin = b["in"]
            nconv = len(convs)
            hw_in = [(h, w)]
            for conv in convs[:-1]:
                d = conv.desc(N, *hw_in[-1])
                hw_in.append((d.OH, d.OW))
            mask = b["mask"].data_ptr()
            yk = next_y()
            y2 = None
            fused_conv3 = False
            shortcut_done = False
            prev_takes_g = False
            if bi > 0 and self.block == "bottleneck":
                pblk = self.blocks[bi - 1]
                if "down_conv" not in pblk:
                    prev_takes_g = True
                else:
                    dp3 = pblk["convs"][-1].desc(N, h, w)
                    prev_takes_g = bool(lib.icamd_conv1x1_bn_bwd_fused_supported(ctypes.byref(dp3)))
            d3 = convs[-1].desc(N, *hw_in[-1])
            fuse3 = (self.block == "bottleneck" and fused_rows > 0
                     and bool(lib.icamd_conv1x1_bn_bwd_fused_supported(ctypes.byref(d3))))

            def fused_conv_bn(conv, bn, dsc, partials, nrows, y_t, x_ptr, dx_ptr, bn_ws, bn_ws_bytes):
                st_ = self.stat_arena.data_ptr() + 4 * bn.stat_offset
                c_ = bn.c
                need = lib.icamd_conv1x1_bn_bwd_fused_workspace_bytes(ctypes.byref(dsc))
                fws = ws.get("fused_ws")
                if fws is None or fws.numel() < need:
                    fws = ws["fused_ws"] = torch.empty(need, dtype=torch.uint8, device=self.device)
                hip.check(lib.icamd_conv1x1_bn_bwd_fused(ctypes.byref(dsc), partials, nrows, dout, y_t.data_ptr(), st_, st_ + 4 * c_,
                                                         st_ + 8 * c_, self._gf(bn.weight), self._gf(bn.bias), x_ptr, self._wt(conv),
                                                         dx_ptr, self._gf(conv.w), acc, bn_ws, bn_ws_bytes, fws.data_ptr(),
                                                         fws.numel(), s), bn.name + " + " + conv.name + " bwd (fused)")

            if "down_conv" in blk and fuse3:
                fused_conv_bn(convs[-1], bns[-1], d3, ws["bnb_part"].data_ptr(), fused_rows, b["y"][-1],
                              b["a"][nconv - 2].data_ptr(), DA, ws["bna_ws"].data_ptr(), ws["bna_ws_bytes"])
                fused_conv3 = True
                dc = blk["down_conv"]
                ddc = dc.desc(N, h, w)
                if dc.stride == 1 and lib.icamd_conv1x1_bn_bwd_fused_supported(ctypes.byref(ddc)):
                    fused_conv_bn(dc, blk["down_bn"], ddc, None, 0, b["yd"], xin.data_ptr(), T, bws, bwb)
                    shortcut_done = True
                else:
                    y2 = next_y()
                    bn_bwd(blk["down_bn"], dout, None, b["yd"], ypool[y2], None, False)
            elif "down_conv" in blk and _DUAL_BNBWD:
                y2 = next_y()
                bnA, bnB = bns[-1], blk["down_bn"]
                stA = self.stat_arena.data_ptr() + 4 * bnA.stat_offset
                stB = self.stat_arena.data_ptr() + 4 * bnB.stat_offset
                c = bnA.c
                hip.check(lib.icamd_bn_bwd_dual(dout, mask, b["y"][-1].data_ptr(), stA, stA + 4 * c, stA + 8 * c,
                                                self._gf(bnA.weight), self._gf(bnA.bias), ypool[yk], b["yd"].data_ptr(), stB,
                                                stB + 4 * c, stB + 8 * c, self._gf(bnB.weight), self._gf(bnB.bias), ypool[y2],
                                                b["y"][-1].numel() // c, c, acc, bws, ws["bnb_ws2"].data_ptr(), bwb, s),
                          bnA.name + " + shortcut bwd")
            elif fused_rows:
                bnl = bns[-1]
                stl = self.stat_arena.data_ptr() + 4 * bnl.stat_offset
                cl = bnl.c
                if fuse3:
                    fused_conv_bn(convs[-1], bnl, d3, ws["bnb_part"].data_ptr(), fused_rows, b["y"][-1],
                                  b["a"][nconv - 2].data_ptr(), DA, ws["bna_ws"].data_ptr(), ws["bna_ws_bytes"])
                    fused_conv3 = True
                else:
                    hip.check(lib.icamd_bn_bwd_from_gy_partials(ws["bnb_part"].data_ptr(), fused_rows, dout, b["y"][-1].data_ptr(),
                                                                stl, stl + 4 * cl, stl + 8 * cl, self._gf(bnl.weight),
                                                                self._gf(bnl.bias), ypool[yk], b["y"][-1].numel() // cl, cl, acc,
                                                                ws["bna_ws"].data_ptr(), ws["bna_ws_bytes"], s),
                              bnl.name + " bwd (apply, sums from the data gradient)")
            else:
                bn_bwd(bns[-1], dout, None, b["y"][-1], ypool[yk], None, True, mask)
            fused_rows = 0
            for i in range(nconv - 1, 0, -1):
                x_i = b["a"][i - 1]
                if fused_conv3 and i == nconv - 1:
                    yk = next_y()
                    bn_bwd(bns[i - 1], DA, None, b["y"][i - 1], ypool[yk], None, True)
                    continue
                wgrad(convs[i], x_i.data_ptr(), ypool[yk], N, *hw_in[i], ybuf=yk)
                dgrad(convs[i], ypool[yk], DA, None, N, *hw_in[i])
                yk = next_y()
                bn_bwd(bns[i - 1], DA, None, b["y"][i - 1], ypool[yk], None, True)
            wgrad(convs[0], xin.data_ptr(), ypool[yk], N, h, w, ybuf=yk)
            if shortcut_done:
                dgrad(convs[0], ypool[yk], other, T, N, h, w)
            elif "down_conv" in blk:
                if y2 is None:
                    y2 = next_y()
                    bn_bwd(blk["down_bn"], dout, None, b["yd"], ypool[y2], None, True, mask)
                dc = blk["down_conv"]
                wgrad(dc, xin.data_ptr(), ypool[y2], N, h, w, ybuf=y2)
                if _SUB2_SHORTCUT and dc.k == 1 and dc.stride == 2 and dc.pad == 0:
                    dd = dc.desc(N, h, w)
                    key = ("sub2", N, dd.OH, dd.OW)
                    d1 = dc.descs.get(key)
                    if d1 is None:
                        d1 = dc.descs[key] = hip.conv_desc(N, dd.OH, dd.OW, dc.cin_p, dc.cout_p, 1, 1, 1, 0)
                    hip.check(lib.icamd_conv2d_dgrad(ctypes.byref(d1), ypool[y2], self._wt(dc), T, None, None, s),
                              dc.name + " dgrad (even grid)")
                    d0 = convs[0].desc(N, h, w)
                    if (prev_takes_g and self.block == "bottleneck"
                            and lib.icamd_conv2d_dgrad_bnred_supported(ctypes.byref(d0))):
                        pb = ws["blocks"][bi - 1]
                        hip.check(lib.icamd_conv2d_dgrad_bnred(ctypes.byref(d0), ypool[yk], self._wt(convs[0]), other, T, None, 1,
                                                               pb["y"][-1].data_ptr(), pb["mask"].data_ptr(),
                                                               ws["bnb_part"].data_ptr(), s),
                                  convs[0].name + " dgrad + shortcut + bn reduce")
                        fused_rows = lib.icamd_conv2d_dgrad_stats_rows(ctypes.byref(d0))
                    else:
                        hip.check(lib.icamd_conv2d_dgrad_sub2(ctypes.byref(d0), ypool[yk], self._wt(convs[0]), other, T, s),
                                  convs[0].name + " dgrad + shortcut")
                else:
                    dgrad(dc, ypool[y2], T, None, N, h, w)
                    dgrad(convs[0], ypool[yk], other, T, N, h, w)
            else:
                d0 = convs[0].desc(N, h, w)
                if (prev_takes_g and self.block == "bottleneck"
                        and lib.icamd_conv2d_dgrad_bnred_supported(ctypes.byref(d0))):
                    pb = ws["blocks"][bi - 1]
                    hip.check(lib.icamd_conv2d_dgrad_bnred(ctypes.byref(d0), ypool[yk], self._wt(convs[0]), other, dout, mask, 0,
                                                           pb["y"][-1].data_ptr(), pb["mask"].data_ptr(),
                                                           ws["bnb_part"].data_ptr(), s), convs[0].name + " dgrad + bn reduce")
                    fused_rows = lib.icamd_conv2d_dgrad_stats_rows(ctypes.byref(d0))
                else:
                    dgrad(convs[0], ypool[yk], other, dout, N, h, w, mask)
            if hook:
                hook(convs[0].w.offset, None, side_events())
            dout, other = other, dout

        d0 = self.stem_conv.desc(N, ws["H"], ws["Ws"])
        yk = next_y()
        if _FUSED_POOL_BWD:
            bn0 = self.stem_bn
            st = self.stat_arena.data_ptr() + 4 * bn0.stat_offset
            c = bn0.c
            hip.check(lib.icamd_bn_bwd_maxpool3x3s2(dout, ws["p0_idx"].data_ptr(), ws["y0"].data_ptr(), st, st + 4 * c,
                                                    st + 8 * c, st + 12 * c, self._gf(bn0.weight), self._gf(bn0.bias),
                                                    ypool[yk], N, d0.OH, d0.OW, c, acc, bws, bwb, s), "stem maxpool + bn bwd")
        else:
            hip.check(lib.icamd_maxpool3x3s2_bwd(dout, ws["p0_idx"].data_ptr(), DA, N, d0.OH, d0.OW, 64, s), "maxpool bwd")
            bn_bwd(self.stem_bn, DA, None, ws["y0"], ypool[yk], None, True)
        wgrad(self.stem_conv, ws["x8"].data_ptr(), ypool[yk], N, ws["H"], ws["Ws"], ybuf=yk)
        for k in range(len(pending)):
            pending[k] = None
        if hook:
            hook(0, None, side_events())
        join_side()

    def _wgrad_stream(self):
        if getattr(self, "_wg_stream", None) is None:
            self._wg_stream = torch.cuda.Stream(device=self.device)
        return self._wg_stream

    def _backward_packed_fused(self, ws, accumulate=False):
        lib = self.lib
        s = hip.stream_ptr()
        N = ws["N"]
        acc = int(bool(accumulate))
        wsp, wsb = ws["wgrad_ws"].data_ptr(), ws["wgrad_ws_bytes"]
        bws, bwb = ws["bnb_ws"].data_ptr(), ws["bnb_ws_bytes"]
        D0, D1, G, T, Y, Y2, DA = (b.data_ptr() for b in self._grad_buffers(ws)[:7])
        hook = self.grad_ready_hook

        def wgrad(conv, x_ptr, dy_ptr, n, ih, iw):
            d = conv.desc(n, ih, iw)
            if conv is self.stem_conv:
                hip.check(lib.icamd_stem7x7s2_wgrad(x_ptr, dy_ptr, self._gf(conv.w), acc, wsp, wsb, n, ih, iw, conv.cout_p, s),
                          conv.name + " wgrad")
                return
            hip.check(lib.icamd_conv2d_wgrad(ctypes.byref(d), x_ptr, dy_ptr, self._gf(conv.w), acc, wsp, wsb, s),
                      conv.name + " wgrad")

        def dgrad(conv, dy_ptr, dx_ptr, addend, n, ih, iw):
            d = conv.desc(n, ih, iw)
            hip.check(lib.icamd_conv2d_dgrad(ctypes.byref(d), dy_ptr, self._wt(conv), dx_ptr, addend, None, s),
                      conv.name + " dgrad")

        def bn_bwd(bn, dout_ptr, act_ptr, y, dy_ptr, gout_ptr, relu):
            st = self.stat_arena.data_ptr() + 4 * bn.stat_offset
            c = bn.c
            rows = y.numel() // c
            hip.check(lib.icamd_bn_bwd(dout_ptr, act_ptr, y.data_ptr(), st, st + 4 * c, st + 8 * c, st + 12 * c,
                                       self._gf(bn.weight), self._gf(bn.bias), dy_ptr, gout_ptr, None, rows, c, int(relu), acc,
                                       bws, bwb, s), bn.name + " bwd")

        P, pw_bytes = ws["bnb_part"].data_ptr(), ws["bna_ws_bytes"]
        aws = ws["bna_ws"].data_ptr()

        def dgrad_bnbwd(conv, dy_ptr, g_ptr, addend, n, ih, iw, bn, y, mask_src, relu):
            d = conv.desc(n, ih, iw)
            st = self.stat_arena.data_ptr() + 4 * bn.stat_offset
            c = bn.c
            f = hip.BnBwdFuse(y.data_ptr(), mask_src, st, st + 4 * c, st + 8 * c, st + 12 * c, P, int(relu))
            hip.check(lib.icamd_conv2d_dgrad_bnbwd(ctypes.byref(d), dy_ptr, self._wt(conv), g_ptr, addend, ctypes.byref(f), s),
                      conv.name + " dgrad+bnbwd")
            return lib.icamd_conv2d_dgrad_stats_rows(ctypes.byref(d))

        def bn_bwd_from_partials(bn, nrows, g_ptr, y, dy_ptr):
            st = self.stat_arena.data_ptr() + 4 * bn.stat_offset
            c = bn.c
            hip.check(lib.icamd_bn_bwd_from_partials(P, nrows, g_ptr, y.data_ptr(), st, st + 4 * c, st + 8 * c,
                                                     self._gf(bn.weight), self._gf(bn.bias), dy_ptr, y.numel() // c, c, acc,
                                                     aws, pw_bytes, s), bn.name + " bwd(apply)")

        dl = ws["dlogits"].data_ptr()
        wgrad(self.fc, ws["pooled"].data_ptr(), dl, N, 1, 1)
        hip.check(lib.icamd_colsum(dl, N, self.ncls_p, self.ncls_p, self._gf(self.fc.b), acc, s), "fc bias grad")
        dgrad(self.fc, dl, ws["dpooled"].data_ptr(), None, N, 1, 1)
        if hook:
            hook(self.fc.w.offset, self.n_params)
        fh, fw = ws["final_hw"]
        dout, other = D0, D1
        hip.check(lib.icamd_avgpool_bwd(ws["dpooled"].data_ptr(), dout, N, fh * fw, self.feat_dim, s), "avgpool bwd")

        nblk = len(self.blocks)
        pending_rows = 0
        for bi in range(nblk - 1, -1, -1):
            blk, b = self.blocks[bi], ws["blocks"][bi]
            convs, bns = blk["convs"], blk["bns"]
            h, w = b["in_hw"]
            xin = b["in"]
            nconv = len(convs)
            hw_in = [(h, w)]
            for conv in convs[:-1]:
                d = conv.desc(N, *hw_in[-1])
                hw_in.append((d.OH, d.OW))
            if bi == nblk - 1:
                bn_bwd(bns[-1], dout, b["a"][-1].data_ptr(), b["y"][-1], Y, G, True)
                g_ptr = G
            else:
                bn_bwd_from_partials(bns[-1], pending_rows, dout, b["y"][-1], Y)
                g_ptr = dout
            for i in range(nconv - 1, 0, -1):
                x_i = b["a"][i - 1]
                wgrad(convs[i], x_i.data_ptr(), Y, N, *hw_in[i])
                nrows = dgrad_bnbwd(convs[i], Y, DA, None, N, *hw_in[i], bns[i - 1], b["y"][i - 1], None, True)
                bn_bwd_from_partials(bns[i - 1], nrows, DA, b["y"][i - 1], Y)
            wgrad(convs[0], xin.data_ptr(), Y, N, h, w)
            if "down_conv" in blk:
                bn_bwd(blk["down_bn"], g_ptr, None, b["yd"], Y2, None, False)
                wgrad(blk["down_conv"], xin.data_ptr(), Y2, N, h, w)
                dgrad(blk["down_conv"], Y2, T, None, N, h, w)
                addend = T
            else:
                addend = g_ptr
            if bi > 0:
                pb, pblk = ws["blocks"][bi - 1], self.blocks[bi - 1]
                pending_rows = dgrad_bnbwd(convs[0], Y, other, addend, N, h, w, pblk["bns"][-1], pb["y"][-1],
                                           xin.data_ptr(), True)
            else:
                dgrad(convs[0], Y, other, addend, N, h, w)
            if hook:
                hook(convs[0].w.offset, None)
            dout, other = other, dout

        d0 = self.stem_conv.desc(N, ws["H"], ws["Ws"])
        hip.check(lib.icamd_maxpool3x3s2_bwd(dout, ws["p0_idx"].data_ptr(), DA, N, d0.OH, d0.OW, 64, s), "maxpool bwd")
        bn_bwd(self.stem_bn, DA, None, ws["y0"], Y, None, True)
        wgrad(self.stem_conv, ws["x8"].data_ptr(), Y, N, ws["H"], ws["Ws"])
        if hook:
            hook(0, None)
```

Before: 14610 images/sec.

## Stage maxpool-bwd gathers in LDS, enable fused pool+BN bwd, tune reductions

Adds dedicated pool-fused BN backward reduce/apply kernels. They stage maxpool dout and index tiles in LDS and pick specialised fixed-window gather paths when a whole wavefront shares the same parity. The fused pool backward becomes the default and the standalone maxpool backward uses the same kernel. Also unrolls the grad-norm sum-of-squares with multiple accumulators, parallelises its finalize across a wave, tiles colsum through shared memory, and adds fastdiv indexing plus vector loads to the input pack kernel. These touch several small kernels plus the stem backward, at the cost of more code, dynamic LDS use and new argument restrictions.

Measured after the change: 14830 images/sec (median of 6 runs). 1.02x the previous value.

```diff
diff --git a/imageclassification_amd/csrc/loss_optim.hip b/imageclassification_amd/csrc/loss_optim.hip
--- a/imageclassification_amd/csrc/loss_optim.hip
+++ b/imageclassification_amd/csrc/loss_optim.hip
@@ -131,11 +131,21 @@
                                                             double* __restrict__ partial) {
   __shared__ double red[4];
   const long long stride = (long long)gridDim.x * blockDim.x;
-  double s = 0.0;
-  for (long long i = (long long)blockIdx.x * blockDim.x + threadIdx.x; i < n4; i += stride) {
+  double acc[4] = {0.0, 0.0, 0.0, 0.0};
+  long long i = (long long)blockIdx.x * blockDim.x + threadIdx.x;
+  for (; i + 3 * stride < n4; i += 4 * stride) {
+    f32x4 v[4];
+#pragma unroll
+    for (int u = 0; u < 4; ++u) v[u] = ((const f32x4*)g)[i + u * stride];
+#pragma unroll
+    for (int u = 0; u < 4; ++u)
+      acc[u] += (double)(v[u][0] * v[u][0] + v[u][1] * v[u][1]) + (double)(v[u][2] * v[u][2] + v[u][3] * v[u][3]);
+  }
+  for (; i < n4; i += stride) {
     const f32x4 v = ((const f32x4*)g)[i];
-    s += (double)(v[0] * v[0] + v[1] * v[1]) + (double)(v[2] * v[2] + v[3] * v[3]);
-  }
+    acc[0] += (double)(v[0] * v[0] + v[1] * v[1]) + (double)(v[2] * v[2] + v[3] * v[3]);
+  }
+  double s = (acc[0] + acc[1]) + (acc[2] + acc[3]);
   if (blockIdx.x == 0 && threadIdx.x == 0)
     for (long long i = n4 * 4; i < n; ++i) s += (double)g[i] * (double)g[i];
   s = wave_sum_d(s);
@@ -146,9 +156,11 @@
 
 __global__ void gradnorm_finalize_kernel(const double* __restrict__ partial, int nblk, float inv_scale, float max_norm,
                                          float* __restrict__ out) {
-  if (threadIdx.x != 0 || blockIdx.x != 0) return;
+  if (blockIdx.x != 0 || threadIdx.x >= 64) return;
   double s = 0.0;
-  for (int i = 0; i < nblk; ++i) s += partial[i];
+  for (int i = (int)threadIdx.x; i < nblk; i += 64) s += partial[i];
+  s = wave_sum_d(s);
+  if (threadIdx.x != 0) return;
   const float norm = (float)sqrt(s) * inv_scale;
   out[0] = norm;
   float coef = 1.f;
@@ -304,11 +316,24 @@
 
 __global__ __launch_bounds__(256) void colsum_kernel(const bf16_t* __restrict__ x, int rows, int ld, int cols,
                                                      float* __restrict__ out, int accumulate) {
-  const int c = blockIdx.x * blockDim.x + threadIdx.x;
-  if (c >= cols) return;
+  __shared__ float tile[64][32];
+  const int cl = threadIdx.x & 31, rl = threadIdx.x >> 5;
+  const int c = blockIdx.x * 32 + cl;
   float s = 0.f;
-  for (int r = 0; r < rows; ++r) s += bf16_to_f32(x[(long long)r * ld + c]);
-  out[c] = accumulate ? out[c] + s : s;
+  for (int r0 = 0; r0 < rows; r0 += 64) {
+#pragma unroll
+    for (int j = 0; j < 8; ++j) {
+      const int r = r0 + rl + 8 * j;
+      tile[rl + 8 * j][cl] = (c < cols && r < rows) ? bf16_to_f32(x[(long long)r * ld + c]) : 0.f;
+    }
+    __syncthreads();
+    if (rl == 0) {
+      const int nr = rows - r0 < 64 ? rows - r0 : 64;
+      for (int k = 0; k < nr; ++k) s += tile[k][cl];
+    }
+    __syncthreads();
+  }
+  if (rl == 0 && c < cols) out[c] = accumulate ? out[c] + s : s;
 }
 
 inline unsigned int grid_for(long long work_items, int threads) {
@@ -468,7 +493,7 @@
 }
 
 int icamd_colsum_launch(const bf16_t* x, int rows, int ld, int cols, float* out, int accumulate, hipStream_t s) {
-  hipLaunchKernelGGL(colsum_kernel, dim3((unsigned)((cols + 255) / 256)), dim3(256), 0, s, x, rows, ld, cols, out,
+  hipLaunchKernelGGL(colsum_kernel, dim3((unsigned)((cols + 31) / 32)), dim3(256), 0, s, x, rows, ld, cols, out,
                      accumulate);
   return icamd_launch_status();
 }
diff --git a/imageclassification_amd/csrc/norm_pool.hip b/imageclassification_amd/csrc/norm_pool.hip
--- a/imageclassification_amd/csrc/norm_pool.hip
+++ b/imageclassification_amd/csrc/norm_pool.hip
@@ -204,14 +204,13 @@
   const unsigned char* idx;
   int IH, IW, OH, OW;
   FastDiv dIW, dIH;
+  int krows;
+  int cap;
 };
 
-__device__ __forceinline__ u32x4 pool_gather8(const bf16_t* __restrict__ dout, const PoolGather& pg, unsigned int row,
+template <class DPtr, class IPtr>
+__device__ __forceinline__ u32x4 pool_gather8(DPtr d8, IPtr i8, unsigned int base, const PoolGather& pg, unsigned int n, int h, int w,
                                               unsigned int cpr, unsigned int cg) {
-  const unsigned int t1 = fdiv(row, pg.dIW);
-  const int w = (int)(row - t1 * pg.IW);
-  const unsigned int n = fdiv(t1, pg.dIH);
-  const int h = (int)(t1 - n * pg.IH);
   float acc[8];
 #pragma unroll
   for (int e = 0; e < 8; ++e) acc[e] = 0.f;
@@ -222,9 +221,9 @@
     for (int ow = ow_lo; ow <= ow_hi; ++ow) {
       if (ow >= pg.OW) continue;
       const unsigned int code4 = (unsigned)(r * 3 + (w - (ow * 2 - 1))) * 0x01010101u;
-      const unsigned int o = ((n * pg.OH + oh) * pg.OW + ow) * cpr + cg;
-      const u32x2 iv = ((const u32x2*)pg.idx)[o];
-      const u32x4 d = ((const u32x4*)dout)[o];
+      const unsigned int o = ((n * pg.OH + oh) * pg.OW + ow) * cpr + cg - base;
+      const u32x2 iv = i8[o];
+      const u32x4 d = d8[o];
       const unsigned int m0 = iv[0] ^ code4, m1 = iv[1] ^ code4;
 #pragma unroll
       for (int e = 0; e < 8; ++e) {
@@ -238,6 +237,63 @@
 #pragma unroll
   for (int e = 0; e < 4; ++e) out[e] = pack_bf16x2(acc[2 * e], acc[2 * e + 1]);
   return out;
+}
+
+template <int NH, int NW, class DPtr, class IPtr>
+__device__ __forceinline__ u32x4 pool_gather8_fixed(DPtr d8, IPtr i8, unsigned int base, const PoolGather& pg, unsigned int n, int h,
+                                                    int w, unsigned int cpr, unsigned int cg) {
+  u32x4 d[NH * NW];
+  u32x2 iv[NH * NW];
+  unsigned int code4[NH * NW];
+#pragma unroll
+  for (int a = 0; a < NH; ++a) {
+#pragma unroll
+    for (int b = 0; b < NW; ++b) {
+      const int oh = (h >> 1) + a, ow = (w >> 1) + b;
+      const bool ok = oh < pg.OH && ow < pg.OW;
+      code4[a * NW + b] = ok ? (unsigned)((h - (oh * 2 - 1)) * 3 + (w - (ow * 2 - 1))) * 0x01010101u : 0x7f7f7f7fu;
+      const unsigned int o = ((n * pg.OH + (ok ? oh : h >> 1)) * pg.OW + (ok ? ow : w >> 1)) * cpr + cg - base;
+      iv[a * NW + b] = i8[o];
+      d[a * NW + b] = d8[o];
+    }
+  }
+  float acc[8];
+#pragma unroll
+  for (int e = 0; e < 8; ++e) acc[e] = 0.f;
+#pragma unroll
+  for (int k = 0; k < NH * NW; ++k) {
+    const unsigned int m0 = iv[k][0] ^ code4[k], m1 = iv[k][1] ^ code4[k];
+#pragma unroll
+    for (int e = 0; e < 8; ++e) {
+      const unsigned int mb = ((e < 4 ? m0 : m1) >> ((e & 3) * 8)) & 0xffu;
+      const float dv = (e & 1) ? bf16_hi(d[k][e >> 1]) : bf16_lo(d[k][e >> 1]);
+      acc[e] += mb == 0u ? dv : 0.f;
+    }
+  }
+  u32x4 out;
+#pragma unroll
+  for (int e = 0; e < 4; ++e) out[e] = pack_bf16x2(acc[2 * e], acc[2 * e + 1]);
+  return out;
+}
+
+__device__ __forceinline__ void bn_bwd_accumulate8(const float (&g)[8], const float (&yy)[8], const float (&mu)[8],
+                                                   const float (&is)[8], float (&sg)[8], float (&sgx)[8]) {
+#pragma unroll
+  for (int e = 0; e < 8; ++e) {
+    sg[e] += g[e];
+    sgx[e] += g[e] * ((yy[e] - mu[e]) * is[e]);
+  }
+}
+__device__ __forceinline__ u32x4 bn_bwd_dy8(const float (&g)[8], const float (&yy)[8], const float (&mu)[8],
+                                            const float (&is)[8], const float (&sc)[8], const float (&k1)[8],
+                                            const float (&k2)[8]) {
+  float o[8];
+#pragma unroll
+  for (int e = 0; e < 8; ++e) o[e] = sc[e] * (g[e] - k1[e] - ((yy[e] - mu[e]) * is[e]) * k2[e]);
+  u32x4 ov;
+#pragma unroll
+  for (int e = 0; e < 4; ++e) ov[e] = pack_bf16x2(o[2 * e], o[2 * e + 1]);
+  return ov;
 }
 
 __global__ __launch_bounds__(256) void bn_bwd_reduce_kernel(const bf16_t* __restrict__ dout, const bf16_t* __restrict__ act,
@@ -245,7 +301,7 @@
                                                             const float* __restrict__ invstd, const float* __restrict__ scale,
                                                             const float* __restrict__ shift, float* __restrict__ part,
                                                             const unsigned char* __restrict__ maskbits, long long rows, int C,
-                                                            int rows_per_block, int relu, const PoolGather pg) {
+                                                            int rows_per_block, int relu) {
   __shared__ float red[256 * 16];
   const int cpr = C >> 3;
   const int tid = threadIdx.x;
@@ -265,8 +321,7 @@
       for (int e = 0; e < 8; ++e) { mu[e] = mean[c + e]; is[e] = invstd[c + e]; sc[e] = scale[c + e]; sh[e] = shift[c + e]; }
       for (long long r = r0 + rl; r < r1; r += rlanes) {
         const long long off = r * cpr + cg0 + cgi;
-        const u32x4 d = pg.idx != nullptr ? pool_gather8(dout, pg, (unsigned)r, (unsigned)cpr, (unsigned)(cg0 + cgi))
-                                          : bn_ld(dout, off);
+        const u32x4 d = bn_ld(dout, off);
         const u32x4 yv = bn_ld(y, off);
         float g[8], yy[8];
 #pragma unroll
@@ -293,11 +348,7 @@
               if (!(fmaf(yy[e], sc[e], sh[e]) > 0.f)) g[e] = 0.f;
           }
         }
-#pragma unroll
-        for (int e = 0; e < 8; ++e) {
-          sg[e] += g[e];
-          sgx[e] += g[e] * ((yy[e] - mu[e]) * is[e]);
-        }
+        bn_bwd_accumulate8(g, yy, mu, is, sg, sgx);
       }
     }
 #pragma unroll
@@ -320,8 +371,7 @@
                                                            const float* __restrict__ shift, const float* __restrict__ c1,
                                                            const float* __restrict__ c2, bf16_t* __restrict__ dy,
                                                            bf16_t* __restrict__ gout, const unsigned char* __restrict__ maskbits,
-                                                           long long nvec, int cpr, int relu, int reverse,
-                                                           const PoolGather pg, const FastDiv dcpr) {
+                                                           long long nvec, int cpr, int relu, int reverse) {
   const long long stride = (long long)gridDim.x * blockDim.x;
   long long k0 = (long long)blockIdx.x * blockDim.x + threadIdx.x;
   const int cg = (int)((reverse ? nvec - 1 - k0 : k0) % cpr) * 8;
@@ -333,13 +383,7 @@
   }
   for (; k0 < nvec; k0 += stride) {
     const long long i = reverse ? nvec - 1 - k0 : k0;
-    u32x4 d;
-    if (pg.idx != nullptr) {
-      const unsigned int row = fdiv((unsigned)i, dcpr);
-      d = pool_gather8(dout, pg, row, (unsigned)cpr, (unsigned)i - row * (unsigned)cpr);
-    } else {
-      d = bn_ld(dout, i);
-    }
+    const u32x4 d = bn_ld(dout, i);
     const u32x4 yv = bn_ld(y, i);
     float g[8], yy[8];
 #pragma unroll
@@ -366,13 +410,7 @@
           if (!(fmaf(yy[e], sc[e], sh[e]) > 0.f)) g[e] = 0.f;
       }
     }
-    float o[8];
-#pragma unroll
-    for (int e = 0; e < 8; ++e) o[e] = sc[e] * (g[e] - k1[e] - ((yy[e] - mu[e]) * is[e]) * k2[e]);
-    u32x4 ov;
-#pragma unroll
-    for (int e = 0; e < 4; ++e) ov[e] = pack_bf16x2(o[2 * e], o[2 * e + 1]);
-    bn_st(dy, i, ov);
+    bn_st(dy, i, bn_bwd_dy8(g, yy, mu, is, sc, k1, k2));
     if (gout != nullptr) {
       u32x4 gv;
 #pragma unroll
@@ -380,6 +418,150 @@
       bn_st(gout, i, gv);
     }
   }
+}
+
+template <int PASS>
+__device__ __forceinline__ void pool_bwd_body(const bf16_t* __restrict__ dout, const bf16_t* __restrict__ y,
+                                              const float* __restrict__ mean, const float* __restrict__ invstd,
+                                              const float* __restrict__ scale, const float* __restrict__ shift,
+                                              const float* __restrict__ c1, const float* __restrict__ c2,
+                                              float* __restrict__ part, bf16_t* __restrict__ out, unsigned int rows, int C,
+                                              unsigned int rows_per_block, const PoolGather& pg) {
+  extern __shared__ __attribute__((aligned(16))) unsigned char pool_smem[];
+  u32x4* sd = (u32x4*)pool_smem;
+  u32x2* si = (u32x2*)(pool_smem + (size_t)pg.cap * 16);
+  const unsigned int cpr = (unsigned)C >> 3;
+  const unsigned int tid = threadIdx.x;
+  const unsigned int rlanes = 256u / cpr;
+  const unsigned int cgi = tid % cpr;
+  unsigned int rl = tid / cpr;
+  if (64u % cpr == 0u && cpr <= 32u) {
+    const unsigned int G = 64u / cpr, wv = tid >> 6, j = (tid & 63u) / cpr;
+    rl = 2u * G * (wv >> 1) + 2u * j + (wv & 1u);
+  }
+  const unsigned int r0 = blockIdx.x * rows_per_block;
+  const unsigned int r1 = (rows - r0 < rows_per_block) ? rows : r0 + rows_per_block;
+  const unsigned int vpr = (unsigned)pg.OW * cpr;
+  float mu[8], is[8], sc[8], sh[8], k1[8], k2[8], sg[8], sgx[8];
+#pragma unroll
+  for (int e = 0; e < 8; ++e) { sg[e] = 0.f; sgx[e] = 0.f; }
+  if constexpr (PASS != 2) {
+    const unsigned int c = cgi * 8;
+#pragma unroll
+    for (int e = 0; e < 8; ++e) { mu[e] = mean[c + e]; is[e] = invstd[c + e]; sc[e] = scale[c + e]; sh[e] = shift[c + e]; }
+    if constexpr (PASS == 1) {
+#pragma unroll
+      for (int e = 0; e < 8; ++e) { k1[e] = c1[c + e]; k2[e] = c2[c + e]; }
+    }
+  }
+  unsigned int r = rl < rlanes ? r0 + rl : r1;
+  for (unsigned int s0 = r0; s0 < r1;) {
+    unsigned int s1 = r1, base = 0;
+    if (pg.krows > 0) {
+      const unsigned int grow = fdiv(s0, pg.dIW);
+      const unsigned int n0 = fdiv(grow, pg.dIH);
+      const unsigned int h0 = grow - n0 * (unsigned)pg.IH;
+      unsigned int hend = h0 + (unsigned)pg.krows;
+      if (hend > (unsigned)pg.IH) hend = (unsigned)pg.IH;
+      const unsigned int send = (n0 * (unsigned)pg.IH + hend) * (unsigned)pg.IW;
+      if (send < s1) s1 = send;
+      unsigned int ohi = hend >> 1;
+      if (ohi > (unsigned)pg.OH - 1u) ohi = (unsigned)pg.OH - 1u;
+      base = (n0 * (unsigned)pg.OH + (h0 >> 1)) * vpr;
+      const unsigned int nv = (ohi - (h0 >> 1) + 1u) * vpr;
+      __syncthreads();
+      for (unsigned int v = tid; v < nv; v += 256u) {
+        sd[v] = ((const u32x4*)dout)[base + v];
+        si[v] = ((const u32x2*)pg.idx)[base + v];
+      }
+      __syncthreads();
+    }
+    unsigned int n = 0;
+    int h = 0, w = 0;
+    if (r < s1) {
+      const unsigned int t1 = fdiv(r, pg.dIW);
+      w = (int)(r - t1 * (unsigned)pg.IW);
+      n = fdiv(t1, pg.dIH);
+      h = (int)(t1 - n * (unsigned)pg.IH);
+    }
+    for (; r < s1; r += rlanes) {
+      u32x4 d;
+      if (pg.krows > 0) {
+        const int key = ((h & 1) << 1) | (w & 1);
+        const int key0 = __builtin_amdgcn_readfirstlane(key);
+        if (__all(key == key0)) {
+          if (key0 == 0) d = pool_gather8_fixed<1, 1>(sd, si, base, pg, n, h, w, cpr, cgi);
+          else if (key0 == 1) d = pool_gather8_fixed<1, 2>(sd, si, base, pg, n, h, w, cpr, cgi);
+          else if (key0 == 2) d = pool_gather8_fixed<2, 1>(sd, si, base, pg, n, h, w, cpr, cgi);
+          else d = pool_gather8_fixed<2, 2>(sd, si, base, pg, n, h, w, cpr, cgi);
+        } else {
+          d = pool_gather8(sd, si, base, pg, n, h, w, cpr, cgi);
+        }
+      } else {
+        d = pool_gather8((const u32x4*)dout, (const u32x2*)pg.idx, 0u, pg, n, h, w, cpr, cgi);
+      }
+      w += (int)rlanes;
+      while (w >= pg.IW) {
+        w -= pg.IW;
+        if (++h == pg.IH) { h = 0; ++n; }
+      }
+      const long long off = (long long)r * cpr + cgi;
+      if constexpr (PASS == 2) {
+        ((u32x4*)out)[off] = d;
+      } else {
+        const u32x4 yv = bn_ld(y, off);
+        float g[8], yy[8];
+#pragma unroll
+        for (int e = 0; e < 4; ++e) {
+          g[2 * e] = bf16_lo(d[e]); g[2 * e + 1] = bf16_hi(d[e]);
+          yy[2 * e] = bf16_lo(yv[e]); yy[2 * e + 1] = bf16_hi(yv[e]);
+        }
+#pragma unroll
+        for (int e = 0; e < 8; ++e)
+          if (!(fmaf(yy[e], sc[e], sh[e]) > 0.f)) g[e] = 0.f;
+        if constexpr (PASS == 0) bn_bwd_accumulate8(g, yy, mu, is, sg, sgx);
+        else bn_st(out, off, bn_bwd_dy8(g, yy, mu, is, sc, k1, k2));
+      }
+    }
+    s0 = s1;
+  }
+  if constexpr (PASS == 0) {
+    float* red = (float*)pool_smem;
+    __syncthreads();
+#pragma unroll
+    for (int e = 0; e < 8; ++e) { red[(rl * cpr + cgi) * 16 + e] = sg[e]; red[(rl * cpr + cgi) * 16 + 8 + e] = sgx[e]; }
+    __syncthreads();
+    for (unsigned int o = tid; o < cpr * 16; o += 256) {
+      const unsigned int cgo = o >> 4, e = o & 15;
+      float s = 0.f;
+      for (unsigned int l = 0; l < rlanes; ++l) s += red[(l * cpr + cgo) * 16 + e];
+      const unsigned int which = e >> 3;
+      part[((long long)blockIdx.x * 2 + which) * C + cgo * 8 + (e & 7)] = s;
+    }
+  }
+}
+
+__global__ __launch_bounds__(256) void bn_bwd_pool_reduce_kernel(const bf16_t* __restrict__ dout, const bf16_t* __restrict__ y,
+                                                                 const float* __restrict__ mean, const float* __restrict__ invstd,
+                                                                 const float* __restrict__ scale, const float* __restrict__ shift,
+                                                                 float* __restrict__ part, unsigned int rows, int C,
+                                                                 unsigned int rows_per_block, const PoolGather pg) {
+  pool_bwd_body<0>(dout, y, mean, invstd, scale, shift, nullptr, nullptr, part, nullptr, rows, C, rows_per_block, pg);
+}
+
+__global__ __launch_bounds__(256) void bn_bwd_pool_apply_kernel(const bf16_t* __restrict__ dout, const bf16_t* __restrict__ y,
+                                                                const float* __restrict__ mean, const float* __restrict__ invstd,
+                                                                const float* __restrict__ scale, const float* __restrict__ shift,
+                                                                const float* __restrict__ c1, const float* __restrict__ c2,
+                                                                bf16_t* __restrict__ dy, unsigned int rows, int C,
+                                                                unsigned int rows_per_block, const PoolGather pg) {
+  pool_bwd_body<1>(dout, y, mean, invstd, scale, shift, c1, c2, nullptr, dy, rows, C, rows_per_block, pg);
+}
+
+__global__ __launch_bounds__(256) void maxpool3x3s2_bwd_kernel(const bf16_t* __restrict__ dout, bf16_t* __restrict__ dx,
+                                                               unsigned int rows, int C, unsigned int rows_per_block,
+                                                               const PoolGather pg) {
+  pool_bwd_body<2>(dout, nullptr, nullptr, nullptr, nullptr, nullptr, nullptr, nullptr, nullptr, dx, rows, C, rows_per_block, pg);
 }
 
 __global__ __launch_bounds__(256) void bn_bwd_dual_reduce_kernel(const bf16_t* __restrict__ dout,
@@ -587,52 +769,6 @@
   }
 }
 
-__global__ __launch_bounds__(256) void maxpool3x3s2_bwd_kernel(const bf16_t* __restrict__ dout,
-                                                               const unsigned char* __restrict__ idx,
-                                                               bf16_t* __restrict__ dx, int N, int IH, int IW, int C,
-                                                               int OH, int OW, const PoolDivs dv) {
-  const unsigned int cpr = (unsigned)C >> 3;
-  const unsigned int total = (unsigned)N * IH * IW * cpr;
-  const unsigned int stride = gridDim.x * blockDim.x;
-  unsigned int i = blockIdx.x * blockDim.x + threadIdx.x;
-  const unsigned int cg = i - fdiv(i, dv.cpr) * cpr;
-  for (; i < total; i += stride) {
-    const unsigned int t = fdiv(i, dv.cpr);
-    const unsigned int t1 = fdiv(t, dv.ow);
-    const int w = (int)(t - t1 * IW);
-    const unsigned int n = fdiv(t1, dv.oh);
-    const int h = (int)(t1 - n * IH);
-    float acc[8];
-#pragma unroll
-    for (int e = 0; e < 8; ++e) acc[e] = 0.f;
-    const int oh_lo = h >> 1, oh_hi = (h + 1) >> 1;
-    const int ow_lo = w >> 1, ow_hi = (w + 1) >> 1;
-    for (int oh = oh_lo; oh <= oh_hi; ++oh) {
-      if (oh >= OH) continue;
-      const int r = h - (oh * 2 - 1);
-      for (int ow = ow_lo; ow <= ow_hi; ++ow) {
-        if (ow >= OW) continue;
-        const int s = w - (ow * 2 - 1);
-        const unsigned int code4 = (unsigned)(r * 3 + s) * 0x01010101u;
-        const unsigned int o = ((n * OH + oh) * OW + ow) * cpr + cg;
-        const u32x2 iv = ((const u32x2*)idx)[o];
-        const u32x4 d = ((const u32x4*)dout)[o];
-        const unsigned int m0 = iv[0] ^ code4, m1 = iv[1] ^ code4;
-#pragma unroll
-        for (int e = 0; e < 8; ++e) {
-          const unsigned int mb = ((e < 4 ? m0 : m1) >> ((e & 3) * 8)) & 0xffu;
-          const float dvv = (e & 1) ? bf16_hi(d[e >> 1]) : bf16_lo(d[e >> 1]);
-          acc[e] += mb == 0u ? dvv : 0.f;
-        }
-      }
-    }
-    u32x4 ov;
-#pragma unroll
-    for (int e = 0; e < 4; ++e) ov[e] = pack_bf16x2(acc[2 * e], acc[2 * e + 1]);
-    ((u32x4*)dx)[i] = ov;
-  }
-}
-
 __global__ __launch_bounds__(256) void avgpool_fwd_kernel(const bf16_t* __restrict__ x, bf16_t* __restrict__ out,
                                                           int N, int HW, int C) {
   const int cpr = C >> 3;
@@ -704,36 +840,53 @@
   }
 }
 
+struct PackDivs { FastDiv wp2, h; };
+typedef float f32x2_a4 __attribute__((ext_vector_type(2), aligned(4)));
+
 __global__ __launch_bounds__(256) void pack_input_rgb4_kernel(const float* __restrict__ x, bf16_t* __restrict__ out, int B,
                                                               int Cin, int H, int W, int mode, float lam, int yl, int yh,
-                                                              int xl, int xh) {
-  const int Wp2 = (W + (W & 1) + 8) / 2;
-  const long long total = (long long)B * H * Wp2;
-  const long long stride = (long long)gridDim.x * blockDim.x;
+                                                              int xl, int xh, const PackDivs dv) {
+  const unsigned int Wp2 = (unsigned)(W + (W & 1) + 8) / 2;
+  const unsigned int total = (unsigned)B * H * Wp2;
+  const unsigned int stride = gridDim.x * blockDim.x;
   const long long hw = (long long)H * W;
-  for (long long i = (long long)blockIdx.x * blockDim.x + threadIdx.x; i < total; i += stride) {
-    const long long row = i / Wp2;
+  for (unsigned int i = blockIdx.x * blockDim.x + threadIdx.x; i < total; i += stride) {
+    const unsigned int row = fdiv(i, dv.wp2);
     const int pp = (int)(i - row * Wp2);
-    const int b = (int)(row / H), h = (int)(row - (long long)b * H);
-    const int fb = B - 1 - b;
+    const unsigned int b = fdiv(row, dv.h);
+    const int h = (int)(row - b * (unsigned)H);
+    const unsigned int fb = (unsigned)B - 1 - b;
+    const int w0 = 2 * pp - 3;
+    const bool in0 = w0 >= 0 && w0 < W, in1 = w0 + 1 >= 0 && w0 + 1 < W;
+    const bool inbox = mode == 2 && h >= yl && h < yh;
+    const bool other = mode == 1 || inbox;
+    const float* pa = x + (long long)b * Cin * hw + (long long)h * W + w0;
+    const float* pb = x + (long long)fb * Cin * hw + (long long)h * W + w0;
     float f[8];
 #pragma unroll
     for (int c = 0; c < 8; ++c) f[c] = 0.f;
 #pragma unroll
-    for (int e = 0; e < 2; ++e) {
-      const int w = 2 * pp + e - 3;
-      if (w >= 0 && w < W) {
-        const long long pix = (long long)h * W + w;
-        for (int c = 0; c < Cin; ++c) {
-          float v = x[((long long)b * Cin + c) * hw + pix];
-          if (mode == 1) {
-            const float o = x[((long long)fb * Cin + c) * hw + pix];
-            v = v * lam + o * (1.f - lam);
-          } else if (mode == 2) {
-            if (h >= yl && h < yh && w >= xl && w < xh) v = x[((long long)fb * Cin + c) * hw + pix];
-          }
-          f[4 * e + c] = v;
+    for (int c = 0; c < 3; ++c) {
+      if (c < Cin) {
+        float v0 = 0.f, v1 = 0.f, o0 = 0.f, o1 = 0.f;
+        if (in0 && in1) {
+          const f32x2_a4 v = *(const f32x2_a4*)(pa + c * hw);
+          v0 = v[0]; v1 = v[1];
+          if (other) { const f32x2_a4 o = *(const f32x2_a4*)(pb + c * hw); o0 = o[0]; o1 = o[1]; }
+        } else {
+          if (in0) { v0 = pa[c * hw]; if (other) o0 = pb[c * hw]; }
+          if (in1) { v1 = pa[c * hw + 1]; if (other) o1 = pb[c * hw + 1]; }
         }
+        if (mode == 1) {
+#pragma clang fp contract(off)
+          v0 = v0 * lam + o0 * (1.f - lam);
+          v1 = v1 * lam + o1 * (1.f - lam);
+        } else if (inbox) {
+          if (w0 >= xl && w0 < xh) v0 = o0;
+          if (w0 + 1 >= xl && w0 + 1 < xh) v1 = o1;
+        }
+        f[c] = in0 ? v0 : 0.f;
+        f[4 + c] = in1 ? v1 : 0.f;
       }
     }
     u32x4 o;
@@ -827,6 +980,19 @@
   return icamd_launch_status();
 }
 
+static PoolGather pool_gather_for(const unsigned char* idx, int IH, int IW, int C, size_t* lds_bytes) {
+  PoolGather pg;
+  memset(&pg, 0, sizeof(pg));
+  pg.idx = idx; pg.IH = IH; pg.IW = IW; pg.OH = (IH - 1) / 2 + 1; pg.OW = (IW - 1) / 2 + 1;
+  pg.dIW = make_fastdiv((unsigned)IW); pg.dIH = make_fastdiv((unsigned)IH);
+  const long long vpr = (long long)pg.OW * (C / 8);
+  for (int k = 4; k >= 2 && pg.krows == 0; k -= 2)
+    if ((k / 2 + 1) * vpr * 24 <= 65536) { pg.krows = k; pg.cap = (int)((k / 2 + 1) * vpr); }
+  const size_t need = (size_t)pg.cap * 24;
+  *lds_bytes = need > 16384 ? need : 16384;
+  return pg;
+}
+
 int icamd_bn_bwd_rows_per_block(long long rows, int C) {
   static const long long nb = []() { const char* e = getenv("ICAMD_BNBWD_BLOCKS"); return e ? atoll(e) : 1024ll; }();
   long long rpb = (rows + nb - 1) / nb;
@@ -841,18 +1007,22 @@
                         double* chunks, float* c1c2, hipStream_t s, const unsigned char* pool_idx, int pool_ih, int pool_iw) {
   if (C % 8 != 0) return ICAMD_ERR_BAD_ARG;
   PoolGather pg;
-  memset(&pg, 0, sizeof(pg));
+  size_t pool_lds = 0;
   if (pool_idx != nullptr) {
-    if (rows * (C / 8) >= (1ll << 31) || pool_ih < 1 || pool_iw < 1 || rows % ((long long)pool_ih * pool_iw) != 0)
+    if (rows * (C / 8) >= (1ll << 31) || pool_ih < 1 || pool_iw < 1 || rows % ((long long)pool_ih * pool_iw) != 0 ||
+        act != nullptr || maskbits != nullptr || gout != nullptr || !relu)
       return ICAMD_ERR_BAD_ARG;
-    pg.idx = pool_idx; pg.IH = pool_ih; pg.IW = pool_iw; pg.OH = (pool_ih - 1) / 2 + 1; pg.OW = (pool_iw - 1) / 2 + 1;
-    pg.dIW = make_fastdiv((unsigned)pool_iw); pg.dIH = make_fastdiv((unsigned)pool_ih);
-  }
-  const FastDiv dcpr = make_fastdiv((unsigned)(C / 8));
+    if (C > 2048) return ICAMD_ERR_UNSUPPORTED;
+    pg = pool_gather_for(pool_idx, pool_ih, pool_iw, C, &pool_lds);
+  }
   const int rpb = icamd_bn_bwd_rows_per_block(rows, C);
   const int nblk = (int)((rows + rpb - 1) / rpb);
-  hipLaunchKernelGGL(bn_bwd_reduce_kernel, dim3((unsigned)nblk), dim3(256), 0, s, dout, act, y, mean, invstd, scale, shift,
-                     part, maskbits, rows, C, rpb, relu, pg);
+  if (pool_idx != nullptr)
+    hipLaunchKernelGGL(bn_bwd_pool_reduce_kernel, dim3((unsigned)nblk), dim3(256), pool_lds, s, dout, y, mean, invstd, scale,
+                       shift, part, (unsigned)rows, C, (unsigned)rpb, pg);
+  else
+    hipLaunchKernelGGL(bn_bwd_reduce_kernel, dim3((unsigned)nblk), dim3(256), 0, s, dout, act, y, mean, invstd, scale, shift,
+                       part, maskbits, rows, C, rpb, relu);
   int rc = icamd_launch_status();
   if (rc) return rc;
   float* c1 = c1c2;
@@ -867,8 +1037,12 @@
     if (rc) return rc;
   }
   const long long nvec = rows * (C / 8);
-  hipLaunchKernelGGL(bn_bwd_apply_kernel, dim3(elementwise_grid(nvec, C / 8)), dim3(256), 0, s, dout, act, y, mean, invstd,
-                     scale, shift, c1, c2, dy, gout, maskbits, nvec, C / 8, relu, bn_reverse(), pg, dcpr);
+  if (pool_idx != nullptr)
+    hipLaunchKernelGGL(bn_bwd_pool_apply_kernel, dim3((unsigned)nblk), dim3(256), pool_lds, s, dout, y, mean, invstd, scale,
+                       shift, c1, c2, dy, (unsigned)rows, C, (unsigned)rpb, pg);
+  else
+    hipLaunchKernelGGL(bn_bwd_apply_kernel, dim3(elementwise_grid(nvec, C / 8)), dim3(256), 0, s, dout, act, y, mean, invstd,
+                       scale, shift, c1, c2, dy, gout, maskbits, nvec, C / 8, relu, bn_reverse());
   return icamd_launch_status();
 }
 
@@ -904,12 +1078,10 @@
 int icamd_bn_bwd_reduce_launch(const bf16_t* g, const bf16_t* y, const float* mean, const float* invstd, float* part, long long rows,
                                int C, int* nblk_out, hipStream_t s) {
   if (C % 8 != 0) return ICAMD_ERR_BAD_ARG;
-  PoolGather pg;
-  memset(&pg, 0, sizeof(pg));
   const int rpb = icamd_bn_bwd_rows_per_block(rows, C);
   const int nblk = (int)((rows + rpb - 1) / rpb);
   hipLaunchKernelGGL(bn_bwd_reduce_kernel, dim3((unsigned)nblk), dim3(256), 0, s, g, (const bf16_t*)nullptr, y, mean, invstd, mean, mean,
-                     part, (const unsigned char*)nullptr, rows, C, rpb, 0, pg);
+                     part, (const unsigned char*)nullptr, rows, C, rpb, 0);
   *nblk_out = nblk;
   return icamd_launch_status();
 }
@@ -944,7 +1116,7 @@
   }
   const long long nvec = rows * (C / 8);
   hipLaunchKernelGGL(bn_bwd_apply_kernel, dim3(elementwise_grid(nvec, C / 8)), dim3(256), 0, s, g, (const bf16_t*)nullptr, y,
-                     mean, invstd, scale, scale, c1, c2, dy, (bf16_t*)nullptr, (const unsigned char*)nullptr, nvec, C / 8, 0, 0, PoolGather{}, make_fastdiv((unsigned)(C / 8)));
+                     mean, invstd, scale, scale, c1, c2, dy, (bf16_t*)nullptr, (const unsigned char*)nullptr, nvec, C / 8, 0, 0);
   return icamd_launch_status();
 }
 
@@ -974,10 +1146,15 @@
 
 int icamd_maxpool_bwd_launch(const bf16_t* dout, const unsigned char* idx, bf16_t* dx, int N, int IH, int IW, int C, int OH,
                              int OW, hipStream_t s) {
-  if (C % 8 != 0 || (long long)N * IH * IW * (C / 8) >= (1ll << 31)) return ICAMD_ERR_BAD_ARG;
-  const long long total = (long long)N * IH * IW * (C / 8);
-  hipLaunchKernelGGL(maxpool3x3s2_bwd_kernel, dim3(elementwise_grid(total, C / 8) * 4), dim3(256), 0, s, dout, idx, dx, N, IH,
-                     IW, C, OH, OW, pool_divs(C, IW, IH));
+  if (C % 8 != 0 || (long long)N * IH * IW * (C / 8) >= (1ll << 31) || OH != (IH - 1) / 2 + 1 || OW != (IW - 1) / 2 + 1)
+    return ICAMD_ERR_BAD_ARG;
+  if (C > 2048) return ICAMD_ERR_UNSUPPORTED;
+  size_t lds = 0;
+  const PoolGather pg = pool_gather_for(idx, IH, IW, C, &lds);
+  const long long rows = (long long)N * IH * IW;
+  const int rpb = icamd_bn_bwd_rows_per_block(rows, C);
+  hipLaunchKernelGGL(maxpool3x3s2_bwd_kernel, dim3((unsigned)((rows + rpb - 1) / rpb)), dim3(256), lds, s, dout, dx,
+                     (unsigned)rows, C, (unsigned)rpb, pg);
   return icamd_launch_status();
 }
 
@@ -1007,10 +1184,14 @@
 
 int icamd_pack_input_rgb4_launch(const float* x, bf16_t* out, int B, int Cin, int H, int W, int mode, float lam, int yl,
                                  int yh, int xl, int xh, hipStream_t s) {
-  if (Cin < 1 || Cin > 3) return ICAMD_ERR_BAD_ARG;
-  const long long total = (long long)B * H * ((W + (W & 1) + 8) / 2);
+  if (Cin < 1 || Cin > 3 || B < 1 || H < 1 || W < 1) return ICAMD_ERR_BAD_ARG;
+  const long long Wp2 = (W + (W & 1) + 8) / 2;
+  const long long total = (long long)B * H * Wp2;
+  if (total >= (1ll << 31)) return ICAMD_ERR_BAD_ARG;
+  PackDivs dv;
+  dv.wp2 = make_fastdiv((unsigned)Wp2); dv.h = make_fastdiv((unsigned)H);
   hipLaunchKernelGGL(pack_input_rgb4_kernel, dim3(grid_for(total, 256, 1) * 2), dim3(256), 0, s, x, out, B, Cin, H, W, mode,
-                     lam, yl, yh, xl, xh);
+                     lam, yl, yh, xl, xh, dv);
   return icamd_launch_status();
 }
 
diff --git a/imageclassification_amd/nets.py b/imageclassification_amd/nets.py
--- a/imageclassification_amd/nets.py
+++ b/imageclassification_amd/nets.py
@@ -13,7 +13,7 @@
 _WGRAD_STREAM = os.environ.get("ICAMD_WGRAD_STREAM", "1") != "0"
 _DUAL_BNBWD = os.environ.get("ICAMD_DUAL_BNBWD", "1") != "0"
 _SUB2_SHORTCUT = os.environ.get("ICAMD_SUB2_SHORTCUT", "1") != "0"
-_FUSED_POOL_BWD = os.environ.get("ICAMD_FUSED_POOL_BWD", "0") == "1"
+_FUSED_POOL_BWD = os.environ.get("ICAMD_FUSED_POOL_BWD", "1") != "0"
 BN_MOMENTUM = 0.1
 
 ARCHS = {
```
